# AlessioSam/LADiff

Hardware: AMD Instinct MI355X
Metric: motions/sec (196-frame, 50-step DDIM, bs128) (higher is better)
Workload: dtype f16x3+f32; 1 GPU; headline:ddim50_cfg7.5_b128_f196_c263_humanml3d; prompts_per_gpu=128, global_batch=128, frames=196, scheduler=ddim, denoising_steps=50, parallelism=dp1, loop=persistent pipeline kernel (16-row blocks x 86)

## Files before the change

ladiff_amd/build.py:

```python
import os
import subprocess
import sys
from concurrent.futures import ThreadPoolExecutor

HERE = os.path.dirname(os.path.abspath(__file__))
CSRC = os.path.join(HERE, "csrc")
OBJ = os.path.join(HERE, "csrc", "build")
LIB = os.path.join(HERE, "libladiff_hip.so")
SOURCES = ["gemm.hip", "gemm_big.hip", "gemm_kr.hip", "gemm_rowln.hip", "rowops.hip", "attention.hip", "qkv_attn.hip", "systolic.hip", "systolic_plan.hip", "linear_ca.hip", "dec_cross.hip", "dec_mlp.hip", "dec_qkv_attn.hip", "feats2joints.hip", "joint_metrics.hip", "vae_losses.hip", "denoiser.hip", "diffusion_stage.hip", "decoder.hip", "encoder.hip", "clip.hip", "evaluator.hip", "reverse.hip", "api.hip"]
FLAGS = ["--offload-arch=gfx950", "-O3", "-std=c++17", "-fPIC", "-fvisibility=hidden", "-Wall", "-Wno-unused-function"]


def _hipcc():
    for c in (os.environ.get("HIPCC"), "/opt/rocm/bin/hipcc", "hipcc"):
        if c and (os.path.isabs(c) and os.path.exists(c) or not os.path.isabs(c)):
            return c
    raise RuntimeError("hipcc not found")


def _stale(target, deps):
    if not os.path.exists(target):
        return True
    t = os.path.getmtime(target)
    return any(os.path.getmtime(d) > t for d in deps)


def stamps_lib(level=1):
    return LIB.replace(".so", "_stamps.so" if int(level) == 1 else f"_stamps{int(level)}.so")


def diag_lib():
    return LIB.replace(".so", "_diag.so")


def build(force=False, verbose=False, stamps=False, tag=None, defines=(), only=None):
    obj, lib, flags = OBJ, LIB, list(FLAGS)
    if tag:
        obj, lib = OBJ + "_" + tag, LIB.replace(".so", f"_{tag}.so")
        flags += ["-D" + d for d in defines]
    if stamps:
        lvl = os.environ.get("LADIFF_STAMPS_LEVEL", "1")
        obj, lib = OBJ + "_stamps" + (lvl if lvl != "1" else ""), stamps_lib(lvl)
        flags.append("-DLADIFF_STAMPS=" + lvl)
    os.makedirs(obj, exist_ok=True)
    headers = [os.path.join(CSRC, f) for f in os.listdir(CSRC) if f.endswith(".h")]
    headers += [os.path.join(os.path.dirname(HERE), "include", h) for h in ("ladiff_hip.h", "ladiff_hip_debug.h")]
    hipcc = _hipcc()
    jobs = []
    objdir = {src: (obj if only is None or src in only else OBJ) for src in SOURCES}
    for src in SOURCES:
        s = os.path.join(CSRC, src)
        o = os.path.join(objdir[src], src.replace(".hip", ".o"))
        if objdir[src] == obj and (force or _stale(o, [s] + headers)):
            jobs.append([hipcc, *flags, "-c", s, "-o", o])

    def run(cmd):
        if verbose:
            print(" ".join(cmd), flush=True)
        r = subprocess.run(cmd, capture_output=True, text=True)
        if r.returncode != 0:
            raise RuntimeError(f"hipcc failed: {' '.join(cmd)}\n{r.stdout}\n{r.stderr}")
        return r.stderr

    with ThreadPoolExecutor(max_workers=4) as ex:
        for err in ex.map(run, jobs):
            if verbose and err.strip():
                print(err)
    objs = [os.path.join(objdir[s], s.replace(".hip", ".o")) for s in SOURCES]
    if force or jobs or _stale(lib, objs + [os.path.join(CSRC, "exports.map")]):
        run([hipcc, "--offload-arch=gfx950", "-shared", "-fPIC", "-fvisibility=hidden", "-Wl,--version-script=" + os.path.join(CSRC, "exports.map"),
             "-o", lib, *objs])
    return lib


def build_all(force=False, verbose=False):
    lib = build(force=force, verbose=verbose)
    build(force=force, verbose=verbose, tag="bf16", defines=["LADIFF_SPLIT_BF16"])
    build(force=force, verbose=verbose, tag="diag", defines=["LADIFF_TAG_BITS=4", "LADIFF_SELFCHECK"], only=("systolic.hip",))
    return lib


if __name__ == "__main__":
    _tag = next((a.split("=", 1)[1] for a in sys.argv if a.startswith("--tag=")), None)
    _defs = [a[2:] for a in sys.argv if a.startswith("-D")]
    if "--all" in sys.argv:
        print(build_all(force="--force" in sys.argv, verbose=True))
    else:
        print(build(force="--force" in sys.argv, verbose=True, stamps="--stamps" in sys.argv, tag=_tag, defines=_defs))
```

ladiff_amd/csrc/api.hip:

```cpp
#include <algorithm>
#include <cstdlib>
#include <cstring>
#include <vector>

#include "model.h"
#include "sampler.h"
#include "../../include/ladiff_hip_debug.h"

using namespace ladiff;

namespace {

inline hipStream_t S(ladiff_stream_t s) { return reinterpret_cast<hipStream_t>(s); }

bool all_set(const float* const* w, size_t n) {
    if (w == nullptr) return false;
    for (size_t i = 0; i < n; ++i)
        if (w[i] == nullptr) return false;
    return true;
}
template <class W>
bool load_weights(W& dst, const float* const* ptrs) {
    if (!all_set(ptrs, sizeof(W) / sizeof(const float*))) return false;
    std::memcpy(&dst, ptrs, sizeof(W));
    return true;
}
const char* name_at(const std::vector<std::string>& n, int i) { return (i >= 0 && i < (int)n.size()) ? n[i].c_str() : nullptr; }

}

#ifdef LADIFF_STAMPS
static unsigned long long* g_stamps = nullptr;
#endif

extern "C" {

int ladiff_version(void) { return LADIFF_ABI_VERSION; }
int ladiff_split_format(void) {
#ifndef LADIFF_SPLIT_BF16
    return 1;
#else
    return 0;
#endif
}

const char* ladiff_error_string(int code) {
    switch (code) {
        case LADIFF_OK: return "ok";
        case LADIFF_ERR_ARG: return "invalid argument (null pointer or negative size)";
        case LADIFF_ERR_SHAPE: return "shape not supported by the gfx950 kernels";
        case LADIFF_ERR_WORKSPACE: return "workspace too small";
        case LADIFF_ERR_UNSUPPORTED: return "configuration branch not built";
        default: return code > 0 ? hipGetErrorString((hipError_t)code) : "unknown ladiff error";
    }
}

int ladiff_denoiser_num_params(void) { return DEN_NPARAMS; }
const char* ladiff_denoiser_param_name(int i) { return name_at(denoiser_param_names(), i); }
int ladiff_decoder_num_params(void) { return DEC_NPARAMS; }
const char* ladiff_decoder_param_name(int i) { return name_at(decoder_param_names(), i); }

int ladiff_gemm(const float* A, int lda, const float* A2, int lda2, int K1, const float* W, int ldw, const float* bias,
                const float* res, int ldres, const float* ln_gamma, const float* ln_beta, float* Y, int ldy, int M,
                int N, int K, int act, ladiff_stream_t stream) {
    LADIFF_CHECK_ARG(A && W && Y && M >= 0 && N > 0 && K > 0);
    GemmArgs g;
    g.A = A; g.lda = lda; g.A2 = A2; g.lda2 = lda2; g.K1 = A2 ? K1 : K; g.W = W; g.ldw = ldw; g.bias = bias;
    g.res = res; g.ldres = ldres; g.ln_g = ln_gamma; g.ln_b = ln_beta; g.Y = Y; g.ldy = ldy; g.M = M; g.N = N; g.K = K;
    g.act = act;
    return launch_gemm(g, S(stream));
}

int ladiff_gemm_resident(const float* A, int lda, const float* A2, int lda2, int K1, const float* W, int ldw,
                         const float* bias, const float* res, int ldres, float* Y, int ldy, int M, int N, int K, int act,
                         int split, float* Ys, ladiff_stream_t stream) {
    LADIFF_CHECK_ARG(A && W && (Y || Ys) && M >= 0 && N > 0 && K > 0);
    if (M == 0) return 0;
    KrArgs g;
    g.A = A; g.lda = lda; g.A2 = A2; g.lda2 = lda2; g.K1 = A2 ? K1 : K; g.W = W; g.ldw = ldw; g.bias = bias;
    g.res = res; g.ldres = ldres; g.Y = Y; g.ldy = ldy; g.M = M; g.N = N; g.K = K; g.act = act;
    g.split = split; g.Ys = Ys;
#ifdef LADIFF_STAMPS
    g.stamps = g_stamps;
#endif
    return launch_gemm_kr(g, S(stream));
}

int ladiff_gemm_split(const float* A, int lda, const float* A2, int lda2, int K1, const float* W, int ldw, const float* bias,
                      const float* res, int ldres, float* Y, float* Ys, int ldy, int M, int N, int K, int act,
                      ladiff_stream_t stream) {
    LADIFF_CHECK_ARG(A && W && (Y || Ys) && M >= 0 && N > 0 && K > 0);
    if (M == 0) return 0;
    GemmArgs g;
    g.A = A; g.lda = lda; g.A2 = A2; g.lda2 = lda2; g.K1 = A2 ? K1 : K; g.W = W; g.ldw = ldw; g.bias = bias;
    g.res = res; g.ldres = ldres; g.Y = Y; g.Ys = Ys; g.ldy = ldy; g.M = M; g.N = N; g.K = K; g.act = act; g.split = 1;
    return launch_gemm(g, S(stream));
}

#ifdef LADIFF_STAMPS
void ladiff_debug_set_stamps(unsigned long long* p) { g_stamps = p; }
void ladiff_debug_set_sys_stamps(unsigned long long* p) { ladiff::g_sys_stamps = p; }
void ladiff_debug_set_probe(int v) { ladiff::g_sys_probe = v; }
#endif

int ladiff_combine_rows(const float* partials, int n_planes, int M, const float* bias, const float* res, int mode,
                        const float* ln_gamma, const float* ln_beta, const float* table, const int32_t* counts, int Bs,
                        int T, int pad_row, float* out, ladiff_stream_t stream) {
    LADIFF_CHECK_ARG(partials && out && n_planes > 0 && M >= 0 && Bs > 0 && T > 0);
    if (mode != RED_PLAIN && mode != RED_LN && mode != RED_LN_ADD && mode != RED_LN_MOD) return LADIFF_ERR_ARG;
    if (mode != RED_PLAIN && !(ln_gamma && ln_beta)) return LADIFF_ERR_ARG;
    if ((mode == RED_LN_ADD || mode == RED_LN_MOD) && !table) return LADIFF_ERR_ARG;
    if (M == 0) return 0;
    return launch_reduce_rows(partials, n_planes, M, bias, res, mode, ln_gamma, ln_beta, table, 0, nullptr, counts, Bs, T,
                              pad_row, 0, out, nullptr, S(stream));
}

int ladiff_layernorm(const float* x, const float* gamma, const float* beta, float* y, int M, ladiff_stream_t stream) {
    LADIFF_CHECK_ARG(x && gamma && beta && y && M >= 0);
    return launch_layernorm(x, gamma, beta, y, M, S(stream));
}

int ladiff_timestep_sinusoid(const int64_t* timesteps, int n, float* out, ladiff_stream_t stream) {
    LADIFF_CHECK_ARG(timesteps && out && n >= 0);
    if (n == 0) return 0;
    return launch_sinusoid(timesteps, n, out, S(stream));
}

int ladiff_decoder_self_attention(const float* qkv, const int32_t* lengths, const uint32_t* keybits, float* out, int B,
                                  int F, ladiff_stream_t stream) {
    LADIFF_CHECK_ARG(qkv && (lengths || keybits) && out && B >= 0);
    return launch_decoder_self_attention(qkv, lengths, keybits, out, B, F, 0, S(stream));
}

int ladiff_self_attention_split(const float* qkv, const int32_t* lengths, const uint32_t* keybits, float* out, int B, int F,
                                 int nheads, int causal, ladiff_stream_t stream) {
    LADIFF_CHECK_ARG(qkv && out && B >= 0);
    return launch_self_attention_split(qkv, lengths, keybits, out, B, F, nheads, causal, 0, S(stream));
}

int ladiff_decoder_cross_attention(const float* q, const float* kv, const int32_t* counts, float* out, int B, int F,
                                   int T, ladiff_stream_t stream) {
    LADIFF_CHECK_ARG(q && kv && out && B >= 0 && F >= 0);
    return launch_decoder_cross_attention(q, kv, counts, out, B, F, T, 0, S(stream));
}

size_t ladiff_denoiser_tables_floats(int n_steps) { return den_tables_floats(n_steps); }
size_t ladiff_denoiser_text_cache_floats(int B2, int n_steps, int n_text) { return den_text_cache_floats(B2, n_steps, n_text); }
size_t ladiff_denoiser_workspace_bytes(int B2, int T, int n_steps, int n_text) {
    return sizeof(float) * std::max({den_forward_ws_floats(B2, T), den_time_layout(nullptr, n_steps).total,
                                     den_text_ws_floats(B2, n_steps, n_text), den_text_ws_floats(B2, n_steps, 1)});
}

int ladiff_denoiser_time_tables(const float* const* w, const float* sinusoid, int n_steps, float* tables, void* ws,
                                size_t ws_bytes, ladiff_stream_t stream) {
    DenoiserW W;
    LADIFF_CHECK_ARG(load_weights(W, w) && sinusoid && tables && ws && n_steps > 0);
    if (ws_bytes < ladiff_denoiser_workspace_bytes(1, 1, n_steps, 1)) return LADIFF_ERR_WORKSPACE;
    return denoiser_time_tables(W, sinusoid, n_steps, tables, (float*)ws, ws_bytes / sizeof(float), S(stream));
}

int ladiff_denoiser_text_cache(const float* const* w, const float* text_emb, int B2, int n_text, const float* tables, int n_steps,
                               float* cache, void* ws, size_t ws_bytes, ladiff_stream_t stream) {
    DenoiserW W;
    LADIFF_CHECK_ARG(load_weights(W, w) && text_emb && tables && cache && ws && B2 > 0 && n_steps > 0 && n_text >= 1);
    if (ws_bytes < ladiff_denoiser_workspace_bytes(B2, 1, n_steps, n_text)) return LADIFF_ERR_WORKSPACE;
    return denoiser_text_cache(W, text_emb, B2, tables, n_steps, cache, (float*)ws, ws_bytes / sizeof(float), S(stream), n_text);
}

int ladiff_denoiser_forward(const float* const* w, const float* const* w_split, const float* tables, const int32_t* d_step,
                            const float* text_cache, int n_text, int n_steps, const float* sample, int Bs, int dup, int T,
                            const int32_t* counts, float* eps, void* ws, size_t ws_bytes, ladiff_stream_t stream) {
    DenoiserW W, WS;
    LADIFF_CHECK_ARG(load_weights(W, w) && tables && d_step && text_cache && sample && eps && ws && Bs > 0 && dup > 0 && n_steps > 0 &&
                     n_text >= 1);
    if (w_split != nullptr) LADIFF_CHECK_ARG(load_weights(WS, w_split));
    if (T < 1 || T > LADIFF_MAX_LATENTS) return LADIFF_ERR_SHAPE;
    if (ws_bytes < ladiff_denoiser_workspace_bytes(Bs * dup, T, n_steps, n_text)) return LADIFF_ERR_WORKSPACE;
    return denoiser_forward(W, w_split ? &WS : nullptr, tables, d_step, text_cache, n_steps, sample, Bs, dup, T, counts, eps, (float*)ws,
                            ws_bytes / sizeof(float), S(stream), 0, -1, 0, n_text);
}

size_t ladiff_linear_cross_attention_workspace_bytes(int B, int T, int n_text) {
    return linear_cross_attention_ws_floats(B, T, n_text) * sizeof(float);
}
int ladiff_linear_cross_attention(const float* const* w, int layer, const float* x, const float* xf, const float* emb,
                                  const int32_t* counts, int B, int T, int n_text, float* out, void* ws, size_t ws_bytes,
                                  ladiff_stream_t stream) {
    DenoiserW W;
    LADIFF_CHECK_ARG(load_weights(W, w) && x && xf && emb && out && ws && B > 0);
    return linear_cross_attention(W, layer, x, xf, emb, counts, B, T, n_text, out, (float*)ws, ws_bytes / sizeof(float), S(stream));
}

int ladiff_cfg_scheduler_step(const float* eps, float* latents, const float* coef, const int32_t* d_step,
                              const float* step_noise, float guidance_scale, int cfg, int B, int T,
                              ladiff_stream_t stream) {
    LADIFF_CHECK_ARG(eps && latents && coef && d_step && B > 0 && T > 0);
    return launch_cfg_step(eps, latents, coef, d_step, step_noise, guidance_scale, cfg, B, T, S(stream));
}
int ladiff_advance_step(int32_t* d_step, ladiff_stream_t stream) {
    LADIFF_CHECK_ARG(d_step);
    return launch_advance(d_step, S(stream));
}
int ladiff_init_latents(const float* noise, const int32_t* counts, float sigma, float* latents, int B, int T,
                        ladiff_stream_t stream) {
    LADIFF_CHECK_ARG(noise && latents && B > 0 && T > 0);
    return launch_init_latents(noise, counts, sigma, latents, B, T, S(stream));
}
int ladiff_finalize_latents(const float* latents, const int32_t* counts, float* z, int B, int T, ladiff_stream_t stream) {
    LADIFF_CHECK_ARG(latents && z && B > 0 && T > 0);
    return launch_finalize_latents(latents, counts, z, B, T, S(stream));
}

int ladiff_sampler_create(void** sampler) {
    LADIFF_CHECK_ARG(sampler);
    *sampler = new Sampler();
    return 0;
}
int ladiff_sampler_destroy(void* sampler) {
    Sampler* sp = reinterpret_cast<Sampler*>(sampler);
    if (sp == nullptr) return 0;
    (void)hipDeviceSynchronize();
    sp->drain_retired();
    if (sp->exec) (void)hipGraphExecDestroy(sp->exec);
    if (sp->setup) (void)hipGraphExecDestroy(sp->setup);
    if (sp->ev0) (void)hipEventDestroy(sp->ev0);
    if (sp->ev1) (void)hipEventDestroy(sp->ev1);
    for (hipEvent_t e : sp->wev) (void)hipEventDestroy(e);
    sp->cap.destroy();
    delete sp;
    return 0;
}

int ladiff_reverse_plan(int B, int T, const int32_t* h_counts, int masked, int loop_mode, int f16x3, int cfg, int* rows_per_block, int* n_blocks) {
    LADIFF_CHECK_ARG(B >= 1 && T >= 1 && T <= LADIFF_MAX_LATENTS && loop_mode >= 1 && loop_mode <= 3 && rows_per_block && n_blocks);
    if (!cfg && masked && h_counts == nullptr) return LADIFF_ERR_UNSUPPORTED;
    std::vector<unsigned char> plan;
    int mr = 2, nb = 0;
    choose_plan(B, T, h_counts, masked != 0, loop_mode, f16x3 != 0, plan, &mr, &nb, cfg != 0);
    *rows_per_block = 16 * mr; *n_blocks = nb;
    return 0;
}

int ladiff_debug_set_stage_waves(int waves_per_simd) {
    LADIFF_CHECK_ARG(waves_per_simd == 1 || waves_per_simd == 2);
    g_waves16 = waves_per_simd;
    return 0;
}

int ladiff_debug_set_handoff(int tagged) {
    LADIFF_CHECK_ARG(tagged == 0 || tagged == 1);
    g_handoff = tagged;
    return 0;
}

int ladiff_debug_set_mlp_variant(int v) {
#ifdef LADIFF_STAMPS
    LADIFF_CHECK_ARG((v >= 0 && v <= 3) || (v >= 11 && v <= 17) || (v >= 21 && v <= 26));
#else
    LADIFF_CHECK_ARG(v >= 0 && v <= 3);
#endif
    g_mlp_variant = v;
    return 0;
}

int ladiff_debug_set_decoder_fusion(int on) {
    LADIFF_CHECK_ARG(on >= 0 && on <= 126 && (on & 3) != 3 && (on & 48) != 48);
    g_dec_out_cross = (on & 64) ? 0 : 1;
    g_dec_fused_mlp = on & 3;
    g_dec_small_rows_path = (on & 4) ? 0 : 1;
    g_dec_final_split = (on & 8) ? 0 : 1;
    g_dec_fused_attn = (on & 16) ? 0 : (on & 32) ? 2 : 1;
    return 0;
}

int ladiff_debug_set_stage_plan(int v) {
    LADIFF_CHECK_ARG(v >= 0 && v <= 1);
    g_stage_plan = v;
    return 0;
}

int ladiff_debug_set_poll_pause(int mask, int len) {
    LADIFF_CHECK_ARG(mask >= 0 && mask <= 255 && len >= 0 && len <= 64);
    g_poll_pause = mask | (len << 8);
    return 0;
}

int ladiff_debug_set_pacing(int eighths, int mask) {
    if (eighths == -1) { g_pace = -1; return 0; }
    LADIFF_CHECK_ARG(eighths >= 0 && eighths <= 8 && mask >= 0 && mask <= 255);
    g_pace = eighths | (mask << 8);
    return 0;
}

int ladiff_debug_set_stage_delay(int mask, int len) {
    LADIFF_CHECK_ARG(mask >= -1 && mask <= 255 && len >= 0 && len <= 64);
    g_stage_delay = mask < 0 ? -1 : (mask | (len << 8));
    return 0;
}

int ladiff_debug_set_loop_thresholds(int look_ahead_from, int small_upto) {
    LADIFF_CHECK_ARG(look_ahead_from >= -1 && small_upto >= -1);
    g_look_ahead_from = look_ahead_from;
    g_small_upto = small_upto;
    return 0;
}

int ladiff_debug_set_graph_epoch_rule(int on) {
    LADIFF_CHECK_ARG(on == 0 || on == 1);
    g_graph_epoch_rule = on;
    return 0;
}

int ladiff_debug_graph_instantiations(void) { return g_graph_instantiations.load(); }

int ladiff_debug_set_xcd_local(int on) {
    LADIFF_CHECK_ARG(on >= 0 && on <= 2);
    g_xcd_local = on;
    return 0;
}

int ladiff_sampler_set_loop(void* sampler, int mode) {
    Sampler* sp = reinterpret_cast<Sampler*>(sampler);
    LADIFF_CHECK_ARG(sp != nullptr && mode >= 0 && mode <= 3);
    sp->loop = mode != 0;
    sp->loop_mode = mode;
    return 0;
}

int ladiff_sampler_loop_ms(void* sampler, float* ms) {
    Sampler* sp = reinterpret_cast<Sampler*>(sampler);
    LADIFF_CHECK_ARG(sp != nullptr && ms != nullptr && sp->ev1 != nullptr);
    LADIFF_HIP(hipEventSynchronize(sp->ev1));
    LADIFF_HIP(hipEventElapsedTime(ms, sp->ev0, sp->ev1));
    return 0;
}

int ladiff_sampler_set_window_timing(void* sampler, int on) {
    Sampler* sp = reinterpret_cast<Sampler*>(sampler);
    LADIFF_CHECK_ARG(sp != nullptr);
    sp->time_windows = on != 0;
    return 0;
}

int ladiff_sampler_window_ms(void* sampler, float* loop_ms_sum, int* n_windows) {
    Sampler* sp = reinterpret_cast<Sampler*>(sampler);
    LADIFF_CHECK_ARG(sp != nullptr && loop_ms_sum != nullptr && n_windows != nullptr);
    float sum = 0.f;
    for (int i = 0; i < sp->n_windows; ++i) {
        float ms = 0.f;
        LADIFF_HIP(hipEventSynchronize(sp->wev[2 * i + 1]));
        LADIFF_HIP(hipEventElapsedTime(&ms, sp->wev[2 * i], sp->wev[2 * i + 1]));
        sum += ms;
    }
    *loop_ms_sum = sum; *n_windows = sp->n_windows;
    return 0;
}

int ladiff_sampler_last_loop(void* sampler, int* pipeline, int* rows_per_block, int* n_blocks) {
    Sampler* sp = reinterpret_cast<Sampler*>(sampler);
    LADIFF_CHECK_ARG(sp != nullptr && pipeline != nullptr);
    *pipeline = sp->last_pipeline;
    if (rows_per_block) *rows_per_block = sp->last_pipeline ? 16 * sp->plan_mr : 0;
    if (n_blocks) *n_blocks = sp->last_pipeline ? sp->plan_nb : 0;
    return 0;
}

int ladiff_sampler_set_noise_generator(void* sampler, uint64_t seed, uint32_t first_prompt, int enable) {
    Sampler* sp = reinterpret_cast<Sampler*>(sampler);
    LADIFF_CHECK_ARG(sp != nullptr);
    sp->gen = NoiseGen{(unsigned)(seed & 0xffffffffull), (unsigned)(seed >> 32), first_prompt, enable ? 1 : 0};
    return 0;
}

int ladiff_noise_fill(uint64_t seed, uint32_t first_prompt, int first_step, int n_steps, int B, int T, float* out, ladiff_stream_t stream) {
    LADIFF_CHECK_ARG(out != nullptr && first_step >= 0 && n_steps >= 0 && B >= 0);
    if (T < 1 || T > LADIFF_MAX_LATENTS) return LADIFF_ERR_SHAPE;
    return launch_noise_fill(NoiseGen{(unsigned)(seed & 0xffffffffull), (unsigned)(seed >> 32), first_prompt, 1}, first_step, n_steps, B, T, out,
                             S(stream));
}

int ladiff_sampler_set_fault(void* sampler, int workgroup, int timeout_ms) {
    Sampler* sp = reinterpret_cast<Sampler*>(sampler);
    LADIFF_CHECK_ARG(sp != nullptr && workgroup >= -1 && workgroup < 256 && timeout_ms >= 0);
    sp->fault_wg = workgroup;
    sp->timeout_ticks = (unsigned long long)timeout_ms * 100000ull;
    return 0;
}

size_t ladiff_reverse_status_offset_bytes(int B, int T, int n_steps, int n_text) {
    if (B < 1 || T < 1 || T > LADIFF_MAX_LATENTS || n_steps < 1 || n_text < 1) return 0;
    const ReverseWs r = carve_reverse(nullptr, B, T, n_steps, n_text);
    return (r.sys_off + sys_status_offset_floats(B, T)) * sizeof(float);
}

int ladiff_reverse_status(void* ws, int B, int T, int n_steps, int n_text, int* code, int* info) {
    LADIFF_CHECK_ARG(ws && code && B > 0 && n_steps > 0);
    if (T < 1 || T > LADIFF_MAX_LATENTS) return LADIFF_ERR_SHAPE;
    const ReverseWs r = carve_reverse(ws, B, T, n_steps, n_text);
    unsigned st[2] = {0u, 0u};
    LADIFF_HIP(hipMemcpy(st, r.sys + sys_status_offset_floats(B, T), sizeof(st), hipMemcpyDeviceToHost));
    *code = (int)st[0];
    if (info) *info = (int)st[1];
    return 0;
}

size_t ladiff_reverse_workspace_bytes(int B, int T, int n_steps, int n_text) { return carve_reverse(nullptr, B, T, n_steps, n_text).total_bytes; }

int ladiff_mlp_ln_fused(const float* xs, const float* x, const float* w1s, const float* b1, const float* w2s, const float* b2,
                        const float* ln_gamma, const float* ln_beta, const float* ln2_gamma, const float* ln2_beta, float* y, float* ys,
                        int M, ladiff_stream_t stream) {
    LADIFF_CHECK_ARG(xs && x && w1s && b1 && w2s && b2 && ln_gamma && ln_beta && (y || ys) && M >= 0);
    if ((ln2_gamma == nullptr) != (ln2_beta == nullptr)) return LADIFF_ERR_ARG;
    return launch_dec_mlp(xs, x, w1s, b1, w2s, b2, ln_gamma, ln_beta, ln2_gamma, ln2_beta, y, ys, M, S(stream));
}

int ladiff_split_rows(const float* x, float* y, int R, int K, ladiff_stream_t stream) {
    LADIFF_CHECK_ARG(x && y && R >= 0 && K > 0);
    if (K % 64) return LADIFF_ERR_SHAPE;
    if (R == 0) return 0;
    return launch_split_rows(x, y, R, K, S(stream));
}

int ladiff_gather_rows(const float* src, const int32_t* index, int n_rows, int row_floats, float* dst, ladiff_stream_t stream) {
    LADIFF_CHECK_ARG(n_rows >= 0 && row_floats > 0);
    if (n_rows == 0) return 0;
    LADIFF_CHECK_ARG(src && index && dst);
    if (row_floats % 4 || (reinterpret_cast<uintptr_t>(src) & 15) || (reinterpret_cast<uintptr_t>(dst) & 15)) return LADIFF_ERR_SHAPE;
    if ((reinterpret_cast<uintptr_t>(index) & 3) || n_rows > (1 << 30)) return LADIFF_ERR_SHAPE;
    return launch_gather_rows(src, index, n_rows, row_floats, dst, S(stream));
}

int ladiff_split_range_stats(const float* const* tensors, const int64_t* counts, int n, int64_t max_count, uint64_t* stats,
                             ladiff_stream_t stream) {
    LADIFF_CHECK_ARG(n >= 0 && max_count >= 0);
    if (n == 0) return 0;
    LADIFF_CHECK_ARG(tensors && counts && stats);
    if (n > 65535 || max_count >= (int64_t(1) << 32)) return LADIFF_ERR_SHAPE;
    return launch_split_range_stats(tensors, counts, n, max_count, reinterpret_cast<unsigned long long*>(stats), S(stream));
}

int ladiff_diffusion_reverse(void* sampler, const float* const* w, const float* const* w_split, uint64_t weights_generation,
                             const float* text_emb, const float* init_noise, const int32_t* counts, const int32_t* final_counts,
                             const int32_t* h_counts, const float* sinusoid, const float* coef, const float* step_noise, float guidance_scale,
                             float init_noise_sigma, int cfg, int B, int T, int n_text, int n_steps, float* z, void* ws, size_t ws_bytes,
                             int reuse_time_tables, ladiff_stream_t stream) {
    DenoiserW W, WS;
    LADIFF_CHECK_ARG(load_weights(W, w) && text_emb && init_noise && sinusoid && coef && z && ws && B > 0 && n_steps > 0);
    if (w_split != nullptr) LADIFF_CHECK_ARG(load_weights(WS, w_split));
    if (T < 1 || T > LADIFF_MAX_LATENTS || n_text < 1) return LADIFF_ERR_SHAPE;
    return diffusion_reverse(reinterpret_cast<Sampler*>(sampler), W, w_split ? &WS : nullptr,
                             ReverseArgs{w, w_split, weights_generation, text_emb, init_noise, counts, final_counts, h_counts, sinusoid, coef,
                                         step_noise, guidance_scale, init_noise_sigma, cfg, B, T, n_text, n_steps, z, ws, ws_bytes,
                                         reuse_time_tables, stream});
}

int ladiff_encoder_num_params(void) { return ENC_NPARAMS; }
const char* ladiff_encoder_param_name(int i) { return name_at(encoder_param_names(), i); }
size_t ladiff_encoder_workspace_bytes(int B, int F, int T, int C) { return enc_ws_floats(B, F, T, C) * sizeof(float); }

int ladiff_vae_encode(const float* const* w, const float* const* w_split, const float* features, const int32_t* lengths,
                      const int32_t* counts, const float* eps, int B, int F, int T, int C, float* mu, float* std,
                      float* latent, void* ws, size_t ws_bytes, ladiff_stream_t stream) {
    EncoderW W, WS;
    LADIFF_CHECK_ARG(load_weights(W, w) && features && lengths && counts && eps && mu && std && latent && ws && B >= 0);
    if (w_split != nullptr) LADIFF_CHECK_ARG(load_weights(WS, w_split));
    return vae_encode(W, w_split ? &WS : nullptr, features, lengths, counts, eps, B, F, T, C, mu, std, latent, (float*)ws,
                      ws_bytes / sizeof(float), S(stream));
}

int ladiff_vae_encode_dvae(const float* const* w, const float* const* w_split, const float* features, const int32_t* lengths,
                           const int32_t* counts, const float* eps, int B, int F, int T, int C, float* mu, float* std, float* latent,
                           void* ws, size_t ws_bytes, const int32_t* slot, const float* values, int n, ladiff_stream_t stream) {
    EncoderW W, WS;
    LADIFF_CHECK_ARG(load_weights(W, w) && features && lengths && counts && eps && mu && std && latent && ws && B >= 0);
    LADIFF_CHECK_ARG(slot && n >= 0 && (values || n == 0));
    if (w_split != nullptr) LADIFF_CHECK_ARG(load_weights(WS, w_split));
    if ((reinterpret_cast<uintptr_t>(slot) & 3) || (reinterpret_cast<uintptr_t>(values) & 3)) return LADIFF_ERR_SHAPE;
    return vae_encode(W, w_split ? &WS : nullptr, features, lengths, counts, eps, B, F, T, C, mu, std, latent, (float*)ws,
                      ws_bytes / sizeof(float), S(stream), slot, values, n);
}

size_t ladiff_vae_losses_workspace_bytes(int B, int F, int C, int J, int T) { return vae_losses_ws_floats(B, F, C, J, T) * sizeof(float); }

int ladiff_vae_losses(const float* m_rst, const float* m_ref, const float* joints_rst, const float* joints_ref, const float* mu,
                      const float* std, int B, int F, int C, int J, int T, double lambda_rec, double lambda_joint, double lambda_kl,
                      double* batch, double* acc, void* ws, size_t ws_bytes, ladiff_stream_t stream) {
    LADIFF_CHECK_ARG(m_rst && m_ref && joints_rst && joints_ref && mu && std && batch && acc && ws);
    if (B < 1 || F < 1 || C < 1 || J < 1 || T < 1) return LADIFF_ERR_SHAPE;
    for (const void* p : {(const void*)m_rst, (const void*)m_ref, (const void*)joints_rst, (const void*)joints_ref, (const void*)mu,
                          (const void*)std})
        if (reinterpret_cast<uintptr_t>(p) & 3) return LADIFF_ERR_SHAPE;
    for (const void* p : {(const void*)batch, (const void*)acc, (const void*)ws})
        if (reinterpret_cast<uintptr_t>(p) & 7) return LADIFF_ERR_SHAPE;
    const VaeLossWs a = vae_losses_layout((float*)ws, B, F, C, J, T);
    if (ws_bytes / sizeof(float) < a.total) return LADIFF_ERR_WORKSPACE;
    return launch_vae_losses(m_rst, m_ref, (size_t)B * F * C, joints_rst, joints_ref, (size_t)B * F * J * 3, mu, std, (size_t)T * B * D,
                             lambda_rec, lambda_joint, lambda_kl, a.part, a.blocks, batch, acc, S(stream));
}

size_t ladiff_denoiser_forward_timesteps_workspace_bytes(int B2, int T) { return den_per_sample_ws_floats(B2, T) * sizeof(float); }

int ladiff_denoiser_forward_timesteps(const float* const* w, const float* const* w_split, const float* text_emb, int n_text,
                                      const int64_t* timesteps, const float* sample, int B2, int T, const int32_t* counts, float* eps,
                                      void* ws, size_t ws_bytes, ladiff_stream_t stream) {
    DenoiserW W, WS;
    LADIFF_CHECK_ARG(load_weights(W, w) && text_emb && timesteps && sample && eps && ws);
    if (w_split != nullptr) LADIFF_CHECK_ARG(load_weights(WS, w_split));
    if (n_text != 1) return LADIFF_ERR_UNSUPPORTED;
    if (B2 < 1 || T < 1 || T > LADIFF_MAX_LATENTS) return LADIFF_ERR_SHAPE;
    for (const void* p : {(const void*)text_emb, (const void*)sample, (const void*)eps, (const void*)ws})
        if (reinterpret_cast<uintptr_t>(p) & 15) return LADIFF_ERR_SHAPE;
    if ((reinterpret_cast<uintptr_t>(timesteps) & 7) || (reinterpret_cast<uintptr_t>(counts) & 3)) return LADIFF_ERR_SHAPE;
    if (ws_bytes < ladiff_denoiser_forward_timesteps_workspace_bytes(B2, T)) return LADIFF_ERR_WORKSPACE;
    return denoiser_forward_timesteps(W, w_split ? &WS : nullptr, text_emb, timesteps, sample, B2, T, counts, eps, (float*)ws,
                                      ws_bytes / sizeof(float), S(stream));
}

int ladiff_q_sample(const float* z, const int64_t* timesteps, const float* alphas_cumprod, int n_train, const int32_t* counts, int draw,
                    uint64_t seed, uint32_t first_prompt, float* noise, float* noisy, int B, int T, ladiff_stream_t stream) {
    LADIFF_CHECK_ARG(z && timesteps && alphas_cumprod && noise && noisy && n_train > 0);
    if (B < 1 || T < 1 || T > LADIFF_MAX_LATENTS) return LADIFF_ERR_SHAPE;
    for (const void* p : {(const void*)z, (const void*)noise, (const void*)noisy})
        if (reinterpret_cast<uintptr_t>(p) & 15) return LADIFF_ERR_SHAPE;
    if ((reinterpret_cast<uintptr_t>(timesteps) & 7) || (reinterpret_cast<uintptr_t>(alphas_cumprod) & 3) ||
        (reinterpret_cast<uintptr_t>(counts) & 3))
        return LADIFF_ERR_SHAPE;
    return launch_q_sample(z, timesteps, alphas_cumprod, n_train, counts,
                           NoiseGen{(unsigned)(seed & 0xffffffffull), (unsigned)(seed >> 32), first_prompt, draw ? 1 : 0}, noise, noisy, B, T,
                           S(stream));
}

size_t ladiff_diffusion_losses_workspace_bytes(int64_t n) { return n < 1 ? 0 : diffusion_losses_layout(nullptr, (size_t)n).total * sizeof(float); }

int ladiff_diffusion_losses(const float* noise_pred, const float* noise, int64_t n, double lambda_inst, double* batch, double* acc, void* ws,
                            size_t ws_bytes, ladiff_stream_t stream) {
    LADIFF_CHECK_ARG(noise_pred && noise && batch && acc && ws);
    if (n < 1) return LADIFF_ERR_SHAPE;
    if ((reinterpret_cast<uintptr_t>(noise_pred) & 3) || (reinterpret_cast<uintptr_t>(noise) & 3)) return LADIFF_ERR_SHAPE;
    for (const void* p : {(const void*)batch, (const void*)acc, (const void*)ws})
        if (reinterpret_cast<uintptr_t>(p) & 7) return LADIFF_ERR_SHAPE;
    const DiffLossWs a = diffusion_losses_layout((float*)ws, (size_t)n);
    if (ws_bytes / sizeof(float) < a.total) return LADIFF_ERR_WORKSPACE;
    return launch_diffusion_losses(noise_pred, noise, (size_t)n, lambda_inst, a.part, a.blocks, batch, acc, S(stream));
}

int ladiff_clip_num_params(void) { return CLIP_NPARAMS; }
const char* ladiff_clip_param_name(int i) { return name_at(clip_param_names(), i); }
size_t ladiff_clip_workspace_bytes(int B, int L) { return clip_ws_floats(B, L) * sizeof(float); }

static bool load_clip(ClipW& dst, const float* const* ptrs, int n_layers) {
    if (ptrs == nullptr || n_layers < 1 || n_layers > CLIP_MAX_LAYERS) return false;
    const int n = CLIP_HEAD_NPARAMS + CLIP_LAYER_NPARAMS * n_layers;
    for (int i = 0; i < n; ++i)
        if (ptrs[i] == nullptr) return false;
    std::memset(&dst, 0, sizeof(dst));
    std::memcpy(&dst, ptrs, n * sizeof(const float*));
    return true;
}

int ladiff_clip_text_encode(const float* const* w, const float* const* w_split, int n_layers, int vocab, const int64_t* ids,
                            int B, int seq, int L, float* out, void* ws, size_t ws_bytes, ladiff_stream_t stream) {
    ClipW W, WS;
    LADIFF_CHECK_ARG(load_clip(W, w, n_layers) && ids && out && ws && B >= 0);
    if (w_split != nullptr) LADIFF_CHECK_ARG(load_clip(WS, w_split, n_layers));
    return clip_text_encode(W, w_split ? &WS : nullptr, n_layers, vocab, ids, B, seq, L, out, (float*)ws,
                            ws_bytes / sizeof(float), S(stream));
}

size_t ladiff_clip_workspace_bytes_ragged(int B, int total_rows) { return clip_ws_floats_rows(B, total_rows) * sizeof(float); }

int ladiff_clip_text_encode_ragged(const float* const* w, const float* const* w_split, int n_layers, int vocab, const int64_t* ids,
                                   int B, int seq, int L, const int32_t* seq_len, const int32_t* row_off, const int32_t* row_seq,
                                   int total_rows, float* out, void* ws, size_t ws_bytes, ladiff_stream_t stream) {
    ClipW W, WS;
    LADIFF_CHECK_ARG(load_clip(W, w, n_layers) && ids && out && ws && B >= 0 && seq_len && row_off && row_seq && total_rows >= 0);
    if (w_split != nullptr) LADIFF_CHECK_ARG(load_clip(WS, w_split, n_layers));
    return clip_text_encode(W, w_split ? &WS : nullptr, n_layers, vocab, ids, B, seq, L, out, (float*)ws,
                            ws_bytes / sizeof(float), S(stream), seq_len, row_off, row_seq, total_rows);
}

int ladiff_t2m_movement_num_params(void) { return (int)t2m_move_param_names().size(); }
const char* ladiff_t2m_movement_param_name(int i) { return name_at(t2m_move_param_names(), i); }
int ladiff_t2m_motion_num_params(void) { return (int)t2m_motion_param_names().size(); }
const char* ladiff_t2m_motion_param_name(int i) { return name_at(t2m_motion_param_names(), i); }
int ladiff_t2m_text_num_params(void) { return (int)t2m_text_param_names().size(); }
const char* ladiff_t2m_text_param_name(int i) { return name_at(t2m_text_param_names(), i); }
size_t ladiff_t2m_movement_workspace_bytes(int B, int F, int Cin) { return t2m_move_ws_floats(B, F, Cin) * sizeof(float); }
size_t ladiff_t2m_motion_workspace_bytes(int B, int T) { return t2m_motion_ws_floats(B, T) * sizeof(float); }
size_t ladiff_t2m_text_workspace_bytes(int B, int L) { return t2m_text_ws_floats(B, L) * sizeof(float); }

int ladiff_t2m_movement_encode(const float* const* w, const float* feats, int ld, int B, int F, int Cin, float* out, void* ws,
                               size_t ws_bytes, ladiff_stream_t stream) {
    LADIFF_CHECK_ARG(all_set(w, t2m_move_param_names().size()) && feats && out && ws && B >= 0);
    return t2m_movement_encode(w, feats, ld, B, F, Cin, out, (float*)ws, ws_bytes / sizeof(float), S(stream));
}
int ladiff_t2m_motion_encode(const float* const* w, const float* movements, const int32_t* m_lens, int B, int T, float* out,
                             void* ws, size_t ws_bytes, ladiff_stream_t stream) {
    LADIFF_CHECK_ARG(all_set(w, t2m_motion_param_names().size()) && movements && m_lens && out && ws && B >= 0);
    return t2m_motion_encode(w, movements, m_lens, B, T, out, (float*)ws, ws_bytes / sizeof(float), S(stream));
}
int ladiff_t2m_text_encode(const float* const* w, const float* word_embs, const float* pos_onehot, const int32_t* cap_lens,
                           int B, int L, float* out, void* ws, size_t ws_bytes, ladiff_stream_t stream) {
    LADIFF_CHECK_ARG(all_set(w, t2m_text_param_names().size()) && word_embs && pos_onehot && cap_lens && out && ws && B >= 0);
    return t2m_text_encode(w, word_embs, pos_onehot, cap_lens, B, L, out, (float*)ws, ws_bytes / sizeof(float), S(stream));
}

int ladiff_feats2joints(const float* feats, const float* mean, const float* std, int B, int F, int C, int njoints,
                        float* joints, ladiff_stream_t stream) {
    LADIFF_CHECK_ARG(feats && mean && std && joints && B >= 0);
    return launch_feats2joints(feats, mean, std, B, F, C, njoints, joints, S(stream));
}

namespace {
int joint_metrics_check(const void* rst, const void* ref, const int32_t* h_lengths, int B, int F, int J, const void* seq_rows, const void* acc) {
    if (J != 21 && J != 22) return LADIFF_ERR_SHAPE;
    if (F < 1 || F > LADIFF_MAX_FRAMES) return LADIFF_ERR_SHAPE;
    for (int b = 0; b < B; ++b)
        if (h_lengths[b] < 1 || h_lengths[b] > F) return LADIFF_ERR_SHAPE;
    if ((reinterpret_cast<uintptr_t>(rst) & 3) || (reinterpret_cast<uintptr_t>(ref) & 3) || (reinterpret_cast<uintptr_t>(seq_rows) & 3) ||
        (reinterpret_cast<uintptr_t>(acc) & 7))
        return LADIFF_ERR_SHAPE;
    return 0;
}
}

int ladiff_joint_ape_ave(const float* joints_rst, const float* joints_ref, const int32_t* lengths, const int32_t* h_lengths, int B, int F,
                         int J, const int32_t* h_part_idx, float factor, float* seq_rows, double* acc, ladiff_stream_t stream) {
    LADIFF_CHECK_ARG(B >= 0);
    if (B == 0) return 0;
    LADIFF_CHECK_ARG(joints_rst && joints_ref && lengths && h_lengths && h_part_idx && seq_rows && acc && factor > 0.f);
    LADIFF_TRY(joint_metrics_check(joints_rst, joints_ref, h_lengths, B, F, J, seq_rows, acc));
    if (reinterpret_cast<uintptr_t>(lengths) & 3) return LADIFF_ERR_SHAPE;
    for (int i = 0; i < 8; ++i)
        if (h_part_idx[i] < 0 || h_part_idx[i] >= (i < 4 ? J - 1 : J)) return LADIFF_ERR_SHAPE;
    return launch_joint_ape_ave(joints_rst, joints_ref, lengths, B, F, J, h_part_idx, factor, seq_rows, acc, S(stream));
}

int ladiff_joint_mr(const float* joints_rst, const float* joints_ref, const int32_t* h_lengths, int B, int F, int J, float* seq_rows,
                    double* acc, ladiff_stream_t stream) {
    LADIFF_CHECK_ARG(B >= 0);
    if (B == 0) return 0;
    LADIFF_CHECK_ARG(joints_rst && joints_ref && h_lengths && seq_rows && acc);
    LADIFF_TRY(joint_metrics_check(joints_rst, joints_ref, h_lengths, B, F, J, seq_rows, acc));
    return launch_joint_mr(joints_rst, joints_ref, B, F, J, seq_rows, acc, S(stream));
}

size_t ladiff_decoder_workspace_bytes(int B, int F, int T, int C) {
    (void)C;
    return dec_ws_floats(B, (size_t)B * F, T) * sizeof(float);
}

int ladiff_vae_decode(const float* const* w, const float* const* w_split, const float* z, const int32_t* lengths,
                      const int32_t* counts, int B, int F, int T, int C, float* feats, void* ws, size_t ws_bytes,
                      ladiff_stream_t stream) {
    DecoderW W, WS;
    LADIFF_CHECK_ARG(load_weights(W, w) && z && lengths && feats && ws && B >= 0);
    if (w_split != nullptr) LADIFF_CHECK_ARG(load_weights(WS, w_split));
    return vae_decode(W, w_split ? &WS : nullptr, z, lengths, counts, nullptr, 0, B, F, T, C, feats, (float*)ws, ws_bytes / sizeof(float),
                      S(stream));
}

namespace {
struct DecodeGraph {
    hipGraphExec_t exec = nullptr;
    GraphSlot slot;
    CaptureStream cap;
};
}

int ladiff_decoder_graph_create(void** graph) {
    LADIFF_CHECK_ARG(graph);
    *graph = new DecodeGraph();
    return 0;
}
int ladiff_decoder_graph_destroy(void* graph) {
    DecodeGraph* g = reinterpret_cast<DecodeGraph*>(graph);
    if (g == nullptr) return 0;
    (void)hipDeviceSynchronize();
    if (g->exec) (void)hipGraphExecDestroy(g->exec);
    g->cap.destroy();
    delete g;
    return 0;
}

int ladiff_vae_decode_graphed(void* graph, const float* const* w, const float* const* w_split, uint64_t weights_generation, const float* z,
                              const int32_t* lengths, const int32_t* counts, const int32_t* row_off, int total_rows, int B, int F, int T,
                              int C, float* feats, void* ws, size_t ws_bytes, ladiff_stream_t stream) {
    DecodeGraph* dg = reinterpret_cast<DecodeGraph*>(graph);
    DecoderW W, WS;
    LADIFF_CHECK_ARG(dg && load_weights(W, w) && z && lengths && feats && ws && B >= 0 && stream != nullptr);
    if (w_split != nullptr) LADIFF_CHECK_ARG(load_weights(WS, w_split));
    if (F < 1 || F > LADIFF_MAX_FRAMES || T < 1 || T > LADIFF_MAX_LATENTS || C < 1) return LADIFF_ERR_SHAPE;
    if (ws_bytes < ladiff_decoder_workspace_bytes(B, F, T, C)) return LADIFF_ERR_WORKSPACE;
    hipStream_t s = S(stream);
    const GraphKey key = decode_key(w, w_split, DEC_NPARAMS, weights_generation, z, lengths, counts, row_off, total_rows, B, F, T, C, feats, ws,
                                    stream, g_dec_fused_mlp, g_dec_small_rows_path, g_dec_final_split, g_mlp_variant, g_dec_fused_attn);
    if (!(dg->exec && dg->slot.key == key && dg->slot.newest())) {
        if (dg->exec) { LADIFF_HIP(hipStreamSynchronize(s)); (void)hipGraphExecDestroy(dg->exec); dg->exec = nullptr; }
        LADIFF_TRY(dec_mlp_prepare());
        LADIFF_TRY(dec_qkv_attn_prepare());
        LADIFF_TRY(dec_cross_prepare());
        LADIFF_TRY(dg->cap.ensure());
        LADIFF_TRY(capture_graph(dg->cap.s, [&](hipStream_t cs) {
            if (row_off != nullptr) LADIFF_TRY(launch_zero_fill(feats, (size_t)B * F * C, cs));
            return vae_decode(W, w_split ? &WS : nullptr, z, lengths, counts, row_off, total_rows, B, F, T, C, feats, (float*)ws,
                              ws_bytes / sizeof(float), cs);
        }, &dg->exec));
        dg->slot.stamp(key);
    }
    LADIFF_HIP(hipGraphLaunch(dg->exec, s));
    return 0;
}

int ladiff_vae_decode_ragged(const float* const* w, const float* const* w_split, const float* z, const int32_t* lengths,
                             const int32_t* counts, const int32_t* row_off, int total_rows, int B, int F, int T, int C, float* feats,
                             void* ws, size_t ws_bytes, ladiff_stream_t stream) {
    DecoderW W, WS;
    LADIFF_CHECK_ARG(load_weights(W, w) && z && lengths && row_off && feats && ws && B >= 0 && total_rows >= 0);
    if (w_split != nullptr) LADIFF_CHECK_ARG(load_weights(WS, w_split));
    if (F < 1 || F > LADIFF_MAX_FRAMES || T < 1 || T > LADIFF_MAX_LATENTS || C < 1) return LADIFF_ERR_SHAPE;
    if (ws_bytes < ladiff_decoder_workspace_bytes(B, F, T, C)) return LADIFF_ERR_WORKSPACE;
    LADIFF_HIP(hipMemsetAsync(feats, 0, (size_t)B * F * C * sizeof(float), S(stream)));
    return vae_decode(W, w_split ? &WS : nullptr, z, lengths, counts, row_off, total_rows, B, F, T, C, feats, (float*)ws,
                      ws_bytes / sizeof(float), S(stream));
}

}
```

ladiff_amd/csrc/dec_cross.hip:

```cpp
#include <mutex>
#include "kernels.h"
#include "tile_mma.h"

namespace ladiff { extern unsigned long long* g_sys_stamps; }

namespace ladiff {

namespace {
constexpr int TM = LADIFF_MAX_LATENTS;
}

__global__ __launch_bounds__(256) void dec_cross_prep_kernel(const DecCrossPrepBatch pb, int B, int T, int tiles_per_wg) {
    const int h = blockIdx.y, layer = blockIdx.z, tid = threadIdx.x, lane = tid & 63, c16 = lane & 15, kq = lane >> 4;
    const int wave = __builtin_amdgcn_readfirstlane(tid >> 6);
    const float* __restrict__ kv = pb.kv[layer]; const float* __restrict__ wq = pb.wq[layer]; const float* __restrict__ bq = pb.bq[layer];
    const float* __restrict__ wo = pb.wo[layer]; float* __restrict__ gu = pb.gu[layer];
    float* __restrict__ cc = gu + (size_t)B * H * T * 2 * D;
    const int M = T * B, ntiles = (M + 15) / 16;
    float gq[4][16], uo[4][16], bqv[16];
#pragma unroll
    for (int t = 0; t < 4; ++t) {
        const int n = 64 * wave + 16 * t + c16;
#pragma unroll
        for (int s = 0; s < 16; ++s) gq[t][s] = wq[(size_t)(h * DH + 16 * kq + s) * D + n];
#pragma unroll
        for (int s4 = 0; s4 < 16; s4 += 4) {
            const f32x4 w4 = ld4(wo + (size_t)n * D + h * DH + 16 * kq + s4);
#pragma unroll
            for (int e = 0; e < 4; ++e) uo[t][s4 + e] = w4[e];
        }
    }
#pragma unroll
    for (int s4 = 0; s4 < 16; s4 += 4) {
        const f32x4 b4 = ld4(bq + h * DH + 16 * kq + s4);
#pragma unroll
        for (int e = 0; e < 4; ++e) bqv[s4 + e] = b4[e];
    }
    const int tile1 = (blockIdx.x + 1) * tiles_per_wg < ntiles ? (blockIdx.x + 1) * tiles_per_wg : ntiles;
    for (int tile = blockIdx.x * tiles_per_wg; tile < tile1; ++tile) {
        const int arow = 16 * tile + c16 < M ? 16 * tile + c16 : M - 1;
        const float* kr = kv + (size_t)arow * 2 * D + h * DH + 16 * kq;
        float ak[16], av[16];
#pragma unroll
        for (int s4 = 0; s4 < 16; s4 += 4) {
            const f32x4 k4 = ld4(kr + s4), v4 = ld4(kr + D + s4);
#pragma unroll
            for (int e = 0; e < 4; ++e) { ak[s4 + e] = k4[e]; av[s4 + e] = v4[e]; }
        }
        f32x4 ag[4], au[4];
#pragma unroll
        for (int t = 0; t < 4; ++t) { ag[t] = f32x4{0.f, 0.f, 0.f, 0.f}; au[t] = ag[t]; }
#pragma unroll
        for (int s = 0; s < 16; ++s)
#pragma unroll
            for (int t = 0; t < 4; ++t) {
                ag[t] = __builtin_amdgcn_mfma_f32_16x16x4f32(ak[s], gq[t][s], ag[t], 0, 0, 0);
                au[t] = __builtin_amdgcn_mfma_f32_16x16x4f32(av[s], uo[t][s], au[t], 0, 0, 0);
            }
#pragma unroll
        for (int i = 0; i < 4; ++i) {
            const int bt = 16 * tile + 4 * kq + i;
            if (bt < M) {
                const int j = bt / B, b = bt - j * B;
                float* o = gu + ((((size_t)b * H + h) * T + j) * 2) * D + 64 * wave + c16;
#pragma unroll
                for (int t = 0; t < 4; ++t) { o[16 * t] = ag[t][i] * 0.125f; o[D + 16 * t] = au[t][i]; }
            }
        }
        if (wave == 0) {
            float c = 0.f;
#pragma unroll
            for (int s = 0; s < 16; ++s) c = fmaf(bqv[s], ak[s], c);
            c += __shfl_xor(c, 16, 64); c += __shfl_xor(c, 32, 64);
            const int bt = 16 * tile + c16;
            if (kq == 0 && bt < M) { const int j = bt / B, b = bt - j * B; cc[((size_t)b * H + h) * T + j] = c * 0.125f; }
        }
    }
}

template <int T>
__device__ __forceinline__ void cross_row(const f32x4 (&xv)[4], f32x4 (&acc)[4], const float* sm, const float* cs, int nv, int c0) {
#pragma unroll 1
    for (int h = 0; h < H; ++h) {
        float sc[T];
#pragma unroll
        for (int j = 0; j < T; ++j) {
            const float* gp = sm + ((size_t)(h * T + j) * 2) * D + c0;
            float d = 0.f;
#pragma unroll
            for (int k = 0; k < 4; ++k) {
                const f32x4 g4 = ld4(gp + 64 * k);
                d = fmaf(xv[k][0], g4[0], fmaf(xv[k][1], g4[1], fmaf(xv[k][2], g4[2], fmaf(xv[k][3], g4[3], d))));
            }
            sc[j] = d;
        }
#pragma unroll
        for (int j = 0; j < T; ++j) sc[j] = row16_sum(sc[j]) + cs[h * T + j];
        float m = -INFINITY;
#pragma unroll
        for (int j = 0; j < T; ++j) { sc[j] = j < nv ? sc[j] : -INFINITY; m = fmaxf(m, sc[j]); }
        float l = 0.f;
#pragma unroll
        for (int j = 0; j < T; ++j) { sc[j] = __builtin_amdgcn_exp2f((sc[j] - m) * 1.4426950408889634f); l += sc[j]; }
        const float inv = 1.f / l;
#pragma unroll
        for (int j = 0; j < T; ++j) {
            const float pj = sc[j] * inv;
            const float* up = sm + ((size_t)(h * T + j) * 2 + 1) * D + c0;
#pragma unroll
            for (int k = 0; k < 4; ++k) {
                const f32x4 u4 = ld4(up + 64 * k);
                acc[k][0] = fmaf(pj, u4[0], acc[k][0]); acc[k][1] = fmaf(pj, u4[1], acc[k][1]);
                acc[k][2] = fmaf(pj, u4[2], acc[k][2]); acc[k][3] = fmaf(pj, u4[3], acc[k][3]);
            }
        }
    }
}

template <int TT>
__global__ __launch_bounds__(256) void dec_cross_apply_kernel(const float* __restrict__ x, const float* __restrict__ gu,
                                                              const float* __restrict__ cc, const int32_t* __restrict__ counts,
                                                              const float* __restrict__ bo, const float* __restrict__ g2,
                                                              const float* __restrict__ b2, int F, int rows_per_wg,
                                                              float* __restrict__ y, float* __restrict__ ys,
                                                              const int32_t* __restrict__ row_off, const float* __restrict__ g1,
                                                              const float* __restrict__ b1) {
    extern __shared__ __attribute__((aligned(16))) float sm[];
    constexpr int T = TT, HT = H * TT;
    const int b = blockIdx.x, tid = threadIdx.x, lane = tid & 63, wave = tid >> 6;
    const float* src = gu + (size_t)b * HT * 2 * D;
    for (int u = tid; u < HT * 2 * D / 4; u += 256) st4(sm + 4 * u, ld4(src + 4 * u));
    float* cs = sm + (size_t)HT * 2 * D;
    if (tid < HT) cs[tid] = cc[(size_t)b * HT + tid];
    int nv = counts != nullptr ? counts[b] : T;
    nv = nv > T ? T : nv;
    __syncthreads();
    const int l16 = lane & 15, grp = lane >> 4, c0 = 4 * l16;
    f32x4 bo4[4], gg[4], bb[4];
#pragma unroll
    for (int k = 0; k < 4; ++k) { bo4[k] = ld4(bo + c0 + 64 * k); gg[k] = ld4(g2 + c0 + 64 * k); bb[k] = ld4(b2 + c0 + 64 * k); }
    size_t row0 = (size_t)b * F;
    if (row_off != nullptr) { row0 = row_off[b]; F = row_off[b + 1] - row_off[b]; }
    const int f0 = blockIdx.y * rows_per_wg;
    const int f1 = f0 + rows_per_wg < F ? f0 + rows_per_wg : F;
    for (int fb = f0; fb < f1; fb += 16) {
        const int f = fb + 4 * wave + grp;
        const bool live = f < f1;
        const size_t row = row0 + (live ? f : f1 - 1);
        f32x4 xv[4], acc[4];
#pragma unroll
        for (int k = 0; k < 4; ++k) xv[k] = ld4(x + row * D + c0 + 64 * k);
        if (g1 != nullptr) {
            float s1 = 0.f;
#pragma unroll
            for (int k = 0; k < 4; ++k) s1 += (xv[k][0] + xv[k][1]) + (xv[k][2] + xv[k][3]);
            const float mean1 = row16_sum(s1) * (1.f / 256.f);
            float q1 = 0.f;
#pragma unroll
            for (int k = 0; k < 4; ++k)
#pragma unroll
                for (int i = 0; i < 4; ++i) { const float dlt = xv[k][i] - mean1; q1 += dlt * dlt; }
            const float rstd1 = rsqrtf(row16_sum(q1) * (1.f / 256.f) + LN_EPS);
#pragma unroll
            for (int k = 0; k < 4; ++k) {
                const f32x4 ga = ld4(g1 + c0 + 64 * k), be = ld4(b1 + c0 + 64 * k);
#pragma unroll
                for (int i = 0; i < 4; ++i) xv[k][i] = (xv[k][i] - mean1) * rstd1 * ga[i] + be[i];
            }
        }
#pragma unroll
        for (int k = 0; k < 4; ++k)
#pragma unroll
            for (int i = 0; i < 4; ++i) acc[k][i] = bo4[k][i] + xv[k][i];
        cross_row<T>(xv, acc, sm, cs, nv, c0);
        float sum = 0.f;
#pragma unroll
        for (int k = 0; k < 4; ++k) sum += (acc[k][0] + acc[k][1]) + (acc[k][2] + acc[k][3]);
        const float mean = row16_sum(sum) * (1.f / 256.f);
        float q = 0.f;
#pragma unroll
        for (int k = 0; k < 4; ++k)
#pragma unroll
            for (int i = 0; i < 4; ++i) { const float dlt = acc[k][i] - mean; q += dlt * dlt; }
        const float rstd = rsqrtf(row16_sum(q) * (1.f / 256.f) + LN_EPS);
        if (live) {
#pragma unroll
            for (int k = 0; k < 4; ++k) {
                f32x4 o;
#pragma unroll
                for (int i = 0; i < 4; ++i) o[i] = (acc[k][i] - mean) * rstd * gg[k][i] + bb[k][i];
                st4(y + row * D + c0 + 64 * k, o);
                if (ys != nullptr) store_split4(ys + row * D, c0 + 64 * k, o);
            }
        }
    }
}


constexpr int OC_ROWS = 32;
constexpr int OC_TILE = OC_ROWS * 1024;
constexpr int OC_CT = OC_ROWS * CLD * 4;
constexpr int OC_XN = OC_ROWS * CLD * 4;
constexpr int OC_SLD = 36;
constexpr int OC_PS = 8 * OC_ROWS * OC_SLD * 4;
constexpr int OC_PT = OC_ROWS * 256;

struct OutCrossArgs {
    const float* att;
    const float* x0;
    const float* wo;
    const float* bo; const float* g1; const float* b1;
    const float* gu; const float* cc;
    const float* bo_c; const float* g2; const float* b2;
    const int32_t* counts; const int32_t* row_off;
    float* y; float* ys;
    int F, rows_per_wg;
    unsigned long long* stamps;
};

#ifdef LADIFF_STAMPS
#define OC_STAMP(i) do { if (p.stamps != nullptr && blockIdx.x == 3 && blockIdx.y == 0 && threadIdx.x == 0 && npass < 6) p.stamps[npass * 16 + (i)] = __builtin_amdgcn_s_memrealtime(); } while (0)
#else
#define OC_STAMP(i) do { } while (0)
#endif

__device__ __forceinline__ void oc_barrier() { asm volatile("s_waitcnt lgkmcnt(0)\n\ts_barrier" ::: "memory"); }

template <int TT>
__global__ __launch_bounds__(512, 1) void dec_out_cross_kernel(const OutCrossArgs p) {
    __shared__ __attribute__((aligned(1024))) char tile[OC_TILE];
    __shared__ __attribute__((aligned(1024))) char ps_b[OC_PS];
    __shared__ __attribute__((aligned(1024))) char ct_b[OC_CT];
    __shared__ __attribute__((aligned(1024))) char xn_b[OC_XN];
    __shared__ __attribute__((aligned(16))) float sc[OC_ROWS * OC_SLD];
    __shared__ __attribute__((aligned(256))) char ptile[OC_PT];
    __shared__ __attribute__((aligned(16))) float vec[6 * D];
    __shared__ float cs[32];
    constexpr int T = TT, HT = H * TT;
    static_assert(HT <= 32, "the (head, token) columns fit one k-step");
    float* ct = reinterpret_cast<float*>(ct_b);
    float* xn = reinterpret_cast<float*>(xn_b);
    float* ps = reinterpret_cast<float*>(ps_b);
    const int b = blockIdx.x, tid = threadIdx.x, lane = tid & 63, frow = lane & 15, fk = lane >> 4;
    const int wave = __builtin_amdgcn_readfirstlane(tid >> 6);
    int npass = 0;
    OC_STAMP(15);
    WFrag<0, 2, 1> gf, uf;
    {
        const float* gub = p.gu + (size_t)b * HT * 2 * D;
#pragma unroll
        for (int j = 0; j < 2; ++j) {
            const int hj = 16 * j + frow;
            f32x4 a = {0.f, 0.f, 0.f, 0.f}, c = a;
            if (hj < HT) { const float* g = gub + (size_t)hj * 2 * D + 32 * wave + 8 * fk; a = ld4(g); c = ld4(g + 4); }
            split8(a, c, gf.hi[j][0], gf.lo[j][0]);
            const int col = 32 * wave + 16 * j + frow;
            f32x4 u0 = {0.f, 0.f, 0.f, 0.f}, u1 = u0;
#pragma unroll
            for (int e = 0; e < 4; ++e) {
                if (8 * fk + e < HT) u0[e] = gub[((size_t)(8 * fk + e) * 2 + 1) * D + col];
                if (8 * fk + 4 + e < HT) u1[e] = gub[((size_t)(8 * fk + 4 + e) * 2 + 1) * D + col];
            }
            split8(u0, u1, uf.hi[j][0], uf.lo[j][0]);
        }
        if (tid < 32) cs[tid] = tid < HT ? p.cc[(size_t)b * HT + tid] : 0.f;
        const float* vs[6] = {p.bo, p.g1, p.b1, p.bo_c, p.g2, p.b2};
        if (tid < 6 * (D / 4)) st4(vec + 4 * tid, ld4(vs[tid / (D / 4)] + 4 * (tid % (D / 4))));
    }
    WFrag<0, 2, 8> wf;
    {
#pragma unroll 1
        for (int half = 0; half < 2; ++half) {
            if (half == 1) __syncthreads();
#pragma unroll
            for (int qq = 0; qq < 4; ++qq) {
                const int q = (qq + b) & 3;
                char* dst = q == 0 ? tile : q == 1 ? ps_b : q == 2 ? ct_b : xn_b;
#pragma unroll
                for (int kk = 0; kk < 4; ++kk) {
                    const int lr32 = wave + 8 * kk, r = 32 * q + lr32;
                    const char* src = reinterpret_cast<const char*>(p.wo) + ((size_t)(128 * half + r) << 10) + ((lane & 48) << 4) + ((((lane & 15) ^ r) & 15) << 4);
                    __builtin_amdgcn_global_load_lds(reinterpret_cast<const float*>(src), (__attribute__((address_space(3))) void*)(dst + lr32 * 1024), 16, 0, 0);
                }
            }
            __builtin_amdgcn_s_waitcnt(0xF70);
            __syncthreads();
            if ((wave >> 2) == half) {
                const int q = wave & 3;
                const char* srcb = q == 0 ? tile : q == 1 ? ps_b : q == 2 ? ct_b : xn_b;
#pragma unroll
                for (int j = 0; j < 2; ++j)
#pragma unroll
                    for (int st = 0; st < 8; ++st) {
                        const int r = 16 * j + frow;
                        wf.hi[j][st] = *reinterpret_cast<const s16x8*>(a_slot<4>(const_cast<char*>(srcb), r, st >> 1, 4 * (st & 1) + fk));
                        wf.lo[j][st] = *reinterpret_cast<const s16x8*>(a_slot<4>(const_cast<char*>(srcb), r, st >> 1, 8 + 4 * (st & 1) + fk));
                    }
            }
        }
        __syncthreads();
    }
    int nv = p.counts != nullptr ? p.counts[b] : T;
    nv = nv > T ? T : nv;
    int F = p.F;
    size_t row0 = (size_t)b * F;
    if (p.row_off != nullptr) { row0 = p.row_off[b]; F = p.row_off[b + 1] - p.row_off[b]; }
    const int f0 = blockIdx.y * p.rows_per_wg;
    const int f1 = f0 + p.rows_per_wg < F ? f0 + p.rows_per_wg : F;
    if (f0 >= f1) return;
    const int l16 = lane & 15, grp = lane >> 4, c0 = 4 * l16, lr = 4 * wave + grp;
    typedef unsigned u32x4_o __attribute__((ext_vector_type(4)));
    const float* x0s = ps;
    auto dma_att = [&](int fb) {
#pragma unroll
        for (int i = 0; i < 4; ++i) {
            const int r = wave + 8 * i, f = fb + r < f1 ? fb + r : f1 - 1;
            unsigned vo = ((lane & 48) << 4) + ((((lane & 15) ^ r) & 15) << 4);
            asm volatile("" : "+v"(vo));
            const char* src = reinterpret_cast<const char*>(p.att) + ((row0 + f) << 10) + vo;
            __builtin_amdgcn_global_load_lds(reinterpret_cast<const float*>(src), (__attribute__((address_space(3))) void*)(tile + r * 1024), 16, 0, 0);
        }
    };
    auto dma_x0 = [&](int fb) {
#pragma unroll
        for (int i = 0; i < 4; ++i) {
            const int r = wave + 8 * i, f = fb + r < f1 ? fb + r : f1 - 1;
            unsigned vo = lane << 4;
            asm volatile("" : "+v"(vo));
            const char* src = reinterpret_cast<const char*>(p.x0) + ((row0 + f) << 10) + vo;
            __builtin_amdgcn_global_load_lds(reinterpret_cast<const float*>(src), (__attribute__((address_space(3))) void*)(ps_b + r * 1024), 16, 0, 0);
        }
    };
    dma_att(f0);
    dma_x0(f0);
    __builtin_amdgcn_s_waitcnt(0xF70);
    __syncthreads();
    for (int fb = f0; fb < f1; fb += OC_ROWS, ++npass) {
        OC_STAMP(0);
        OC_STAMP(1);
        f32x4 acc2[2][2];
        zero_acc(acc2);
        mma<0, 4, 2, 8, 2>(tile, wf, acc2);
        OC_STAMP(2);
        const int f = fb + lr;
        const bool live = f < f1;
        const size_t row = row0 + (live ? f : f1 - 1);
        f32x4 xv[4];
        stage_c(ct, acc2, [&](int j) { return 32 * wave + 16 * j; });
        __builtin_amdgcn_s_waitcnt(0xF70);
        __syncthreads();
        OC_STAMP(3);
        {
            const float* cr = ct + lr * CLD + c0;
#pragma unroll
            for (int k = 0; k < 4; ++k) {
                const f32x4 o = ld4(cr + 64 * k), bo = ld4(vec + c0 + 64 * k), r0 = ld4(x0s + lr * D + c0 + 64 * k);
#pragma unroll
                for (int i = 0; i < 4; ++i) xv[k][i] = (o[i] + bo[i]) + r0[i];
            }
            float s1 = 0.f;
#pragma unroll
            for (int k = 0; k < 4; ++k) s1 += (xv[k][0] + xv[k][1]) + (xv[k][2] + xv[k][3]);
            const float mean1 = row16_sum(s1) * (1.f / 256.f);
            float q1 = 0.f;
#pragma unroll
            for (int k = 0; k < 4; ++k)
#pragma unroll
                for (int i = 0; i < 4; ++i) { const float dlt = xv[k][i] - mean1; q1 += dlt * dlt; }
            const float rstd1 = rsqrtf(row16_sum(q1) * (1.f / 256.f) + LN_EPS);
#pragma unroll
            for (int k = 0; k < 4; ++k) {
                const f32x4 ga = ld4(vec + D + c0 + 64 * k), be = ld4(vec + 2 * D + c0 + 64 * k);
#pragma unroll
                for (int i = 0; i < 4; ++i) xv[k][i] = (xv[k][i] - mean1) * rstd1 * ga[i] + be[i];
                st4(xn + lr * CLD + c0 + 64 * k, xv[k]);
                tile_put4<0, 4>(tile, lr, c0 + 64 * k, xv[k]);
            }
        }
        OC_STAMP(4);
        __syncthreads();
        OC_STAMP(5);
        {
            u32x4_o ah[2], al[2];
#pragma unroll
            for (int i = 0; i < 2; ++i) {
                ah[i] = *reinterpret_cast<const u32x4_o*>(a_slot<4>(tile, 16 * i + frow, wave >> 1, 4 * (wave & 1) + fk));
                al[i] = *reinterpret_cast<const u32x4_o*>(a_slot<4>(tile, 16 * i + frow, wave >> 1, 8 + 4 * (wave & 1) + fk));
            }
            f32x4 as[2][2];
            zero_acc(as);
#pragma unroll
            for (int i = 0; i < 2; ++i)
#pragma unroll
                for (int j = 0; j < 2; ++j) as[i][j] = MFMA16_S16(__builtin_bit_cast(s16x8, al[i]), gf.hi[j][0], as[i][j], 0, 0, 0);
#pragma unroll
            for (int i = 0; i < 2; ++i)
#pragma unroll
                for (int j = 0; j < 2; ++j) as[i][j] = MFMA16_S16(__builtin_bit_cast(s16x8, ah[i]), gf.lo[j][0], as[i][j], 0, 0, 0);
#pragma unroll
            for (int i = 0; i < 2; ++i)
#pragma unroll
                for (int j = 0; j < 2; ++j) as[i][j] = MFMA16_S16(__builtin_bit_cast(s16x8, ah[i]), gf.hi[j][0], as[i][j], 0, 0, 0);
            float* pw = ps + wave * (OC_ROWS * OC_SLD);
#pragma unroll
            for (int i = 0; i < 2; ++i)
#pragma unroll
                for (int j = 0; j < 2; ++j)
#pragma unroll
                    for (int r = 0; r < 4; ++r) pw[(16 * i + 4 * fk + r) * OC_SLD + 16 * j + frow] = as[i][j][r];
        }
        __syncthreads();
        OC_STAMP(6);
        if (fb + OC_ROWS < f1) dma_att(fb + OC_ROWS);
        {
            float tot[2];
#pragma unroll
            for (int u = 0; u < 2; ++u) {
                const int hj = 16 * u + l16;
                float a = 0.f;
#pragma unroll
                for (int w = 0; w < 8; ++w) a += ps[w * (OC_ROWS * OC_SLD) + lr * OC_SLD + hj];
                tot[u] = a + cs[hj];
                sc[lr * OC_SLD + hj] = tot[u];
            }
            asm volatile("s_waitcnt lgkmcnt(0)" ::: "memory");
            __builtin_amdgcn_wave_barrier();
            float hs[2][T];
            int hh[2], jj[2];
#pragma unroll
            for (int u = 0; u < 2; ++u) {
                const int hj = 16 * u + l16;
                hh[u] = hj < HT ? hj / T : 0; jj[u] = hj - hh[u] * T;
#pragma unroll
                for (int t = 0; t < T; ++t) hs[u][t] = sc[lr * OC_SLD + hh[u] * T + t];
            }
#pragma unroll
            for (int u = 0; u < 2; ++u) {
                const int hj = 16 * u + l16;
                float m = -INFINITY, l = 0.f;
#pragma unroll
                for (int t = 0; t < T; ++t) m = t < nv ? fmaxf(m, hs[u][t]) : m;
#pragma unroll
                for (int t = 0; t < T; ++t) l += t < nv ? __builtin_amdgcn_exp2f((hs[u][t] - m) * 1.4426950408889634f) : 0.f;
                float pr = __builtin_amdgcn_exp2f((tot[u] - m) * 1.4426950408889634f) / l;
                if (!(hj < HT && jj[u] < nv)) pr = 0.f;
                tile_put1<0, 1>(ptile, lr, hj, pr);
            }
        }
        oc_barrier();
        OC_STAMP(7);
        f32x4 ao[2][2];
        zero_acc(ao);
        mma<0, 1, 2, 1, 2>(ptile, uf, ao);
        stage_c(ct, ao, [&](int j) { return 32 * wave + 16 * j; });
        __builtin_amdgcn_s_waitcnt(0xF70);
        oc_barrier();
        OC_STAMP(8);
        {
            const float* cr = ct + lr * CLD + c0;
            f32x4 acc[4];
#pragma unroll
            for (int k = 0; k < 4; ++k) {
                const f32x4 o = ld4(cr + 64 * k), bc = ld4(vec + 3 * D + c0 + 64 * k), x1 = ld4(xn + lr * CLD + c0 + 64 * k);
#pragma unroll
                for (int i = 0; i < 4; ++i) acc[k][i] = (bc[i] + x1[i]) + o[i];
            }
            if (fb + OC_ROWS < f1) dma_x0(fb + OC_ROWS);
            float sum = 0.f;
#pragma unroll
            for (int k = 0; k < 4; ++k) sum += (acc[k][0] + acc[k][1]) + (acc[k][2] + acc[k][3]);
            const float mean = row16_sum(sum) * (1.f / 256.f);
            float q = 0.f;
#pragma unroll
            for (int k = 0; k < 4; ++k)
#pragma unroll
                for (int i = 0; i < 4; ++i) { const float dlt = acc[k][i] - mean; q += dlt * dlt; }
            const float rstd = rsqrtf(row16_sum(q) * (1.f / 256.f) + LN_EPS);
            if (live) {
#pragma unroll
                for (int k = 0; k < 4; ++k) {
                    const f32x4 ga = ld4(vec + 4 * D + c0 + 64 * k), be = ld4(vec + 5 * D + c0 + 64 * k);
                    f32x4 o;
#pragma unroll
                    for (int i = 0; i < 4; ++i) o[i] = (acc[k][i] - mean) * rstd * ga[i] + be[i];
                    st4(p.y + row * D + c0 + 64 * k, o);
                    if (p.ys != nullptr) store_split4(p.ys + row * D, c0 + 64 * k, o);
                }
            }
        }
        OC_STAMP(9);
    }
}

int dec_cross_prepare() {
    static std::mutex mu;
    static bool attr_set[64] = {};
    int dev = 0;
    LADIFF_HIP(hipGetDevice(&dev));
    if (dev < 0 || dev >= 64) return LADIFF_ERR_ARG;
    std::lock_guard<std::mutex> lock(mu);
    if (!attr_set[dev]) {
        LADIFF_HIP(hipFuncSetAttribute(reinterpret_cast<const void*>(dec_cross_apply_kernel<8>), hipFuncAttributeMaxDynamicSharedMemorySize,
                                       (int)(((size_t)H * TM * 2 * D + H * TM) * sizeof(float))));
        const void* oc[8] = {reinterpret_cast<const void*>(dec_out_cross_kernel<1>), reinterpret_cast<const void*>(dec_out_cross_kernel<2>),
                             reinterpret_cast<const void*>(dec_out_cross_kernel<3>), reinterpret_cast<const void*>(dec_out_cross_kernel<4>),
                             reinterpret_cast<const void*>(dec_out_cross_kernel<5>), reinterpret_cast<const void*>(dec_out_cross_kernel<6>),
                             reinterpret_cast<const void*>(dec_out_cross_kernel<7>), reinterpret_cast<const void*>(dec_out_cross_kernel<8>)};
        for (int t = 1; t <= 8; ++t)
            (void)oc[t - 1];
        attr_set[dev] = true;
    }
    return 0;
}

int launch_decoder_cross_prep(const DecCrossPrepBatch& pb, int n, int B, int T, hipStream_t s) {
    if (B == 0 || n == 0) return 0;
    if (T < 1 || T > TM || n > DEC_PREP_MAX) return LADIFF_ERR_SHAPE;
    const int ntiles = (T * B + 15) / 16;
    int tpw = 1;
    while (tpw < 8 && (ntiles + 2 * tpw - 1) / (2 * tpw) * H * n >= 160) tpw *= 2;
    hipLaunchKernelGGL(dec_cross_prep_kernel, dim3((ntiles + tpw - 1) / tpw, H, n), dim3(256), 0, s, pb, B, T, tpw);
    LADIFF_LAUNCH_CHECK();
    return 0;
}

int launch_decoder_cross_apply(const float* x, const float* bo, const float* g2, const float* b2, const int32_t* counts, int B, int F,
                               int T, const float* gu_ws, float* y, float* ys, hipStream_t s, const int32_t* row_off, const float* g1,
                               const float* b1) {
    if (B == 0 || F == 0) return 0;
    if (T < 1 || T > TM) return LADIFF_ERR_SHAPE;
    const float* gu = gu_ws;
    const float* cc = gu_ws + (size_t)B * H * T * 2 * D;
    int chunks = (512 + B - 1) / B;
    if (chunks < 1) chunks = 1;
    if (chunks > (F + 3) / 4) chunks = (F + 3) / 4;
    const int rows_per_wg = ((F + chunks - 1) / chunks + 15) / 16 * 16;
    chunks = (F + rows_per_wg - 1) / rows_per_wg;
    const size_t lds = ((size_t)H * T * 2 * D + H * T) * sizeof(float);
    LADIFF_TRY(dec_cross_prepare());
#define LADIFF_DC_CASE(TT)                                                                                                   \
    case TT:                                                                                                                 \
        hipLaunchKernelGGL(dec_cross_apply_kernel<TT>, dim3(B, chunks), dim3(256), lds, s, x, gu, cc, counts, bo, g2, b2, F, \
                           rows_per_wg, y, ys, row_off, g1, b1);                                                                              \
        break;
    switch (T) {
        LADIFF_DC_CASE(1) LADIFF_DC_CASE(2) LADIFF_DC_CASE(3) LADIFF_DC_CASE(4)
        LADIFF_DC_CASE(5) LADIFF_DC_CASE(6) LADIFF_DC_CASE(7) LADIFF_DC_CASE(8)
        default: return LADIFF_ERR_SHAPE;
    }
#undef LADIFF_DC_CASE
    LADIFF_LAUNCH_CHECK();
    return 0;
}

int launch_decoder_out_cross(const float* att_s, const float* x0, const float* wo_s, const float* bo, const float* g1, const float* b1,
                             const float* bo_c, const float* g2, const float* b2, const int32_t* counts, int B, int F, int T,
                             const float* gu_ws, float* y, float* ys, hipStream_t s, const int32_t* row_off) {
    if (B == 0 || F == 0) return 0;
    if (T < 1 || T > TM) return LADIFF_ERR_SHAPE;
    int chunks = (256 + B - 1) / B;
    if (chunks > (F + OC_ROWS - 1) / OC_ROWS) chunks = (F + OC_ROWS - 1) / OC_ROWS;
    if (chunks < 1) chunks = 1;
    const int rows_per_wg = ((F + chunks - 1) / chunks + OC_ROWS - 1) / OC_ROWS * OC_ROWS;
    chunks = (F + rows_per_wg - 1) / rows_per_wg;
    LADIFF_TRY(dec_cross_prepare());
    OutCrossArgs a{att_s, x0, wo_s, bo, g1, b1, gu_ws, gu_ws + (size_t)B * H * T * 2 * D, bo_c, g2, b2, counts, row_off, y, ys, F, rows_per_wg, nullptr};
#ifdef LADIFF_STAMPS
    a.stamps = g_sys_stamps;
#endif
#define LADIFF_OC_CASE(TT) \
    case TT: hipLaunchKernelGGL(dec_out_cross_kernel<TT>, dim3(B, chunks), dim3(512), 0, s, a); break;
    switch (T) {
        LADIFF_OC_CASE(1) LADIFF_OC_CASE(2) LADIFF_OC_CASE(3) LADIFF_OC_CASE(4)
        LADIFF_OC_CASE(5) LADIFF_OC_CASE(6) LADIFF_OC_CASE(7) LADIFF_OC_CASE(8)
        default: return LADIFF_ERR_SHAPE;
    }
#undef LADIFF_OC_CASE
    LADIFF_LAUNCH_CHECK();
    return 0;
}

}
```

ladiff_amd/csrc/dec_mlp.hip:

```cpp
#include <mutex>
#include "model.h"
#include "tile_mma.h"

namespace ladiff {

namespace {

constexpr int MLP_NS = 8;
constexpr int MLP_GRP = 4;
constexpr int MLP_STAGE = 16384;
constexpr int MLP_LDS = MLP_NS * MLP_STAGE + FF * 4 + 5 * D * 4;

typedef unsigned u32x4_m __attribute__((ext_vector_type(4)));

struct MlpArgs {
    const float* xs;
    const float* x;
    const float* w1;
    const float* b1;
    const float* w2;
    const float* b2;
    const float* g3; const float* be3;
    const float* g4; const float* be4;
    float* y; float* ys;
    int M;
};

__device__ __forceinline__ int pi_row(int p) { const int j = p >> 4, n = p & 15; return 32 * (j >> 1) + 8 * (n >> 2) + 4 * (j & 1) + (n & 3); }

template <int N> __device__ __forceinline__ void wait_vm() { asm volatile("s_waitcnt vmcnt(%0)" ::"n"(N) : "memory"); }
template <int OFF>
__device__ __forceinline__ void fetch16(u32x4_m& v, unsigned addr) {
    asm volatile("ds_read_b128 %0, %1 offset:%2" : "=v"(v) : "v"(addr), "n"(OFF) : "memory");
}
template <int OFF>
__device__ __forceinline__ void fetch16_keep(u32x4_m& v, unsigned addr) {
    asm volatile("ds_read_b128 %0, %1 offset:%2" : "+v"(v) : "v"(addr), "n"(OFF) : "memory");
}
template <int N>
__device__ __forceinline__ void wait_lgkm(u32x4_m& a, u32x4_m& b, u32x4_m& c, u32x4_m& d) {
    asm volatile("s_waitcnt lgkmcnt(%4)" : "+v"(a), "+v"(b), "+v"(c), "+v"(d) : "n"(N));
}
__device__ __forceinline__ s16x8 as_bf(const u32x4_m v) { return __builtin_bit_cast(s16x8, v); }

}

template <int NW, int RT, int DIAG = 0>
__global__ __launch_bounds__(64 * NW, NW / 4) void dec_mlp_kernel(const MlpArgs p) {
    constexpr int NT = 64 * NW, RW = 16 * RT, BM = RW * NW, PPW = 16 / NW;
    extern __shared__ __attribute__((aligned(1024))) char lds[];
    float* const b1s = reinterpret_cast<float*>(lds + MLP_NS * MLP_STAGE);
    const int tid = threadIdx.x, lane = tid & 63;
    const int wave = __builtin_amdgcn_readfirstlane(tid >> 6);
    const int frow = lane & 15, fk = lane >> 4;
    const int M = p.M;
    int myrow[RT]; bool live[RT];
#pragma unroll
    for (int rt = 0; rt < RT; ++rt) {
        myrow[rt] = blockIdx.x * BM + RW * wave + 16 * rt + frow;
        live[rt] = myrow[rt] < M;
        myrow[rt] = live[rt] ? myrow[rt] : M - 1;
    }

    s16x8 xh[RT][8], xl[RT][8];
#pragma unroll
    for (int rt = 0; rt < RT; ++rt) {
        const char* xr = reinterpret_cast<const char*>(p.xs) + (size_t)myrow[rt] * 1024 + fk * 16;
#pragma unroll
        for (int s = 0; s < 8; ++s) {
            xh[rt][s] = *reinterpret_cast<const s16x8*>(xr + (s >> 1) * 256 + (s & 1) * 64);
            xl[rt][s] = *reinterpret_cast<const s16x8*>(xr + (s >> 1) * 256 + (s & 1) * 64 + 128);
        }
    }
    for (int i = tid; i < FF / 4; i += NT) st4(b1s + 4 * i, ld4(p.b1 + 4 * i));
    float* const prm = b1s + FF;
    for (int i = tid; i < 5 * D / 4; i += NT) {
        const int which = i / (D / 4), c4 = i % (D / 4);
        const float* src = which == 0 ? p.b2 : which == 1 ? p.g3 : which == 2 ? p.be3 : which == 3 ? p.g4 : p.be4;
        if (src != nullptr) st4(prm + 4 * i, ld4(src + 4 * c4));
    }

    const int cs = (lane & 7) ^ ((lane >> 4) & 3) ^ (4 * (wave & 1));
    const int koff = (cs < 4 ? cs * 4 : 32 + (cs - 4) * 4);
    int src[PPW];
#pragma unroll
    for (int i = 0; i < PPW; ++i) src[i] = pi_row(8 * (wave + NW * i) + (lane >> 3));
    char* const dma_dst = lds + (8 * wave) * 128;
    auto issue = [&](int hs, auto uc, auto slotc, auto ic) __attribute__((always_inline)) {
        constexpr int u = decltype(uc)::value, slot = decltype(slotc)::value, i = decltype(ic)::value;
        const float* base; int ldw, n0, kb, half;
        const int hsv = hs < 0 ? 0 : hs;
        if constexpr (u < 8) { base = p.w1; ldw = D; n0 = 128 * hsv; kb = u >> 1; half = u & 1; }
        else { constexpr int v = u - 8, c = v >> 1; base = p.w2; ldw = FF; n0 = 128 * (v & 1); kb = 2 * hsv + (c >> 1); half = c & 1; }
        const float* s0 = base + (size_t)(n0 + src[i]) * ldw + kb * 64 + half * 16 + koff;
        if constexpr (DIAG == 1) { if (hs >= 0) return; }
        __builtin_amdgcn_global_load_lds(s0, (__attribute__((address_space(3))) void*)(dma_dst + slot * MLP_STAGE + 8 * NW * i * 128), 16, 0, 0);
    };

    const int sw = (frow >> 1) & 7;
    const unsigned rd_hi = lds_addr(lds) + frow * 128 + ((fk ^ sw) << 4);
    const unsigned rd_lo = lds_addr(lds) + frow * 128 + (((4 + fk) ^ sw) << 4);
    const unsigned rd_hi2 = rd_hi + 4 * MLP_STAGE, rd_lo2 = rd_lo + 4 * MLP_STAGE;

    f32x4 hacc[RT][8], oacc[RT][16];
    s16x8 hh[RT][4], hl[RT][4];
#pragma unroll
    for (int rt = 0; rt < RT; ++rt)
#pragma unroll
        for (int j = 0; j < 16; ++j) oacc[rt][j] = f32x4{0.f, 0.f, 0.f, 0.f};

    u32x4_m wt[4][2];
    u32x4_m dummy[4][2];
    if constexpr (DIAG == 3 || DIAG == 6 || DIAG == 7) {
#pragma unroll
        for (int i = 0; i < 4; ++i) { asm volatile("" : "=v"(wt[i][0])); asm volatile("" : "=v"(wt[i][1])); asm volatile("" : "=v"(dummy[i][0])); asm volatile("" : "=v"(dummy[i][1])); }
    }
    auto fetch_tile = [&](auto slotc, auto jc) __attribute__((always_inline)) {
        constexpr int slot = decltype(slotc)::value, j = decltype(jc)::value;
        if constexpr (DIAG == 3) return;
        const unsigned ah = slot < 4 ? rd_hi : rd_hi2, al = slot < 4 ? rd_lo : rd_lo2;
        constexpr int so = (slot & 3) * MLP_STAGE;
        if constexpr (DIAG == 6) { fetch16_keep<so + j * 2048>(dummy[j & 3][0], ah); fetch16_keep<so + j * 2048>(dummy[j & 3][1], al); return; }
        fetch16<so + j * 2048>(wt[j & 3][0], ah); fetch16<so + j * 2048>(wt[j & 3][1], al);
    };
    auto stage_mma = [&](auto slotc, auto& acc, auto j0c, const s16x8 (&bh)[RT], const s16x8 (&bl)[RT], auto&& between, auto&& next) __attribute__((always_inline)) {
        constexpr int slot = decltype(slotc)::value, J0 = decltype(j0c)::value;
        static_for<8>([&](auto jc) {
            constexpr int j = decltype(jc)::value, cur = j & 3;
            next(jc);
            if constexpr (DIAG != 3 && DIAG != 6) asm volatile("s_waitcnt lgkmcnt(4)" : "+v"(wt[cur][0]), "+v"(wt[cur][1]));
            __builtin_amdgcn_sched_barrier(0);
            static_for<3 * RT>([&](auto mc) {
                constexpr int m = decltype(mc)::value, prod = m / RT, rt = m % RT;
                if constexpr (DIAG == 7) {
                    acc[rt][J0 + j] = MFMA16_S16(as_bf(dummy[cur][prod == 1]), prod == 0 ? bl[rt] : bh[rt], acc[rt][J0 + j], 0, 0, 0);
                } else if constexpr (DIAG != 2) {
                    if constexpr (prod == 0) acc[rt][J0 + j] = MFMA16_S16(as_bf(wt[cur][0]), bl[rt], acc[rt][J0 + j], 0, 0, 0);
                    else if constexpr (prod == 1) acc[rt][J0 + j] = MFMA16_S16(as_bf(wt[cur][1]), bh[rt], acc[rt][J0 + j], 0, 0, 0);
                    else acc[rt][J0 + j] = MFMA16_S16(as_bf(wt[cur][0]), bh[rt], acc[rt][J0 + j], 0, 0, 0);
                }
                if constexpr (m == 0) {
                    __builtin_amdgcn_sched_barrier(0);
                    if constexpr (j + 3 < 8) fetch_tile(slotc, IntC<j + 3>{});
                    else fetch_tile(IntC<(slot + 1) % MLP_NS>{}, IntC<j + 3 - 8>{});
                    __builtin_amdgcn_sched_barrier(0);
                }
            });
            if constexpr (DIAG == 2) acc[0][J0 + j][0] += __builtin_bit_cast(float, wt[cur][0][0]) + __builtin_bit_cast(float, wt[cur][1][1]);
            __builtin_amdgcn_sched_barrier(0);
            if constexpr (j & 1) between(IntC<j / 2>{});
        });
    };

    static_for<MLP_GRP>([&](auto uc) {
        constexpr int u = decltype(uc)::value;
        static_for<PPW>([&](auto ic) { issue(DIAG == 1 ? -1 : 0, IntC<u>{}, IntC<u>{}, ic); });
    });
    __syncthreads();
    auto landed = [&]() __attribute__((always_inline)) {
        wait_vm<0>();
        __builtin_amdgcn_s_barrier();
    };
    landed();
    static_for<PPW>([&](auto ic) { issue(DIAG == 1 ? -1 : 0, IntC<MLP_GRP>{}, IntC<MLP_GRP>{}, ic); });
    static_for<3>([&](auto jc) { fetch_tile(IntC<0>{}, jc); });
    constexpr int H = PPW / 2;
#pragma unroll 1
    for (int hs = 0; hs < 8; ++hs) {
        static_for<16>([&](auto uc) {
            constexpr int u = decltype(uc)::value, slot = u % MLP_NS, r = u % MLP_GRP;
            auto batch_pieces = [&](auto aheadc, auto halfc) __attribute__((always_inline)) {
                constexpr int ahead = decltype(aheadc)::value, half = decltype(halfc)::value;
                constexpr int ut = (u + ahead) % 16, slot_t = (u + ahead) % MLP_NS;
                const int hs_t = (hs + (u + ahead >= 16 ? 1 : 0)) & 7;
                static_for<H>([&](auto ic) { issue(hs_t, IntC<ut>{}, IntC<slot_t>{}, IntC<H * half + decltype(ic)::value>{}); });
            };
            auto between = [&](auto gc) __attribute__((always_inline)) {
                constexpr int g = decltype(gc)::value;
                if constexpr (r == 3 && g >= 2) batch_pieces(IntC<5>{}, IntC<g - 2>{});
                else if constexpr (r == 0 && g < 2) batch_pieces(IntC<5>{}, IntC<g>{});
                else if constexpr (r == 0 && g >= 2) batch_pieces(IntC<6>{}, IntC<g - 2>{});
                else if constexpr (r == 1 && g < 2) batch_pieces(IntC<6>{}, IntC<g>{});
            };
            auto next = [&](auto jc) __attribute__((always_inline)) {
                constexpr int j = decltype(jc)::value;
                if constexpr (r == 3 && j == 5) landed();
                else if constexpr (r == 0 && j == 5) __builtin_amdgcn_s_barrier();
            };
            if constexpr (u < 8) {
                if constexpr (u == 0) {
#pragma unroll
                    for (int rt = 0; rt < RT; ++rt)
#pragma unroll
                        for (int j = 0; j < 8; ++j) hacc[rt][j] = f32x4{0.f, 0.f, 0.f, 0.f};
                }
                s16x8 bh[RT], bl[RT];
#pragma unroll
                for (int rt = 0; rt < RT; ++rt) { bh[rt] = xh[rt][u]; bl[rt] = xl[rt][u]; }
                stage_mma(IntC<slot>{}, hacc, IntC<0>{}, bh, bl, between, next);
            } else {
                constexpr int v = u - 8, c = v >> 1, nh = v & 1;
                if constexpr (nh == 0) {
                    const f32x4 ba = ld4(b1s + 128 * hs + 32 * c + 8 * fk), bb = ld4(b1s + 128 * hs + 32 * c + 8 * fk + 4);
#pragma unroll
                    for (int rt = 0; rt < RT; ++rt) {
                        f32x4 va, vb;
#pragma unroll
                        for (int e = 0; e < 4; ++e) {
                            if constexpr (DIAG == 4) { va[e] = hacc[rt][2 * c][e] + ba[e]; vb[e] = hacc[rt][2 * c + 1][e] + bb[e]; }
                            else { va[e] = gelu_erf(hacc[rt][2 * c][e] + ba[e]); vb[e] = gelu_erf(hacc[rt][2 * c + 1][e] + bb[e]); }
                        }
                        split8(va, vb, hh[rt][c], hl[rt][c]);
                    }
                }
                s16x8 bh[RT], bl[RT];
#pragma unroll
                for (int rt = 0; rt < RT; ++rt) { bh[rt] = hh[rt][c]; bl[rt] = hl[rt][c]; }
                stage_mma(IntC<slot>{}, oacc, IntC<8 * nh>{}, bh, bl, between, next);
            }
        });
    }
    wait_vm<0>();
    if constexpr (DIAG == 6) {
        wait_lgkm<0>(dummy[0][0], dummy[0][1], dummy[1][0], dummy[1][1]);
        wait_lgkm<0>(dummy[2][0], dummy[2][1], dummy[3][0], dummy[3][1]);
    } else if constexpr (DIAG != 3) {
        wait_lgkm<0>(wt[0][0], wt[0][1], wt[1][0], wt[1][1]);
        wait_lgkm<0>(wt[2][0], wt[2][1], wt[3][0], wt[3][1]);
    }

    if constexpr (DIAG == 5) {
        float s = 0.f;
#pragma unroll
        for (int rt = 0; rt < RT; ++rt)
#pragma unroll
            for (int jj = 0; jj < 16; ++jj) s += oacc[rt][jj][0] + oacc[rt][jj][1] + oacc[rt][jj][2] + oacc[rt][jj][3];
        if (live[0] && p.y != nullptr) p.y[(size_t)myrow[0] * D + fk] = s;
        return;
    }
    __syncthreads();
    char* const stg = lds + wave * 16384;
#pragma unroll
    for (int rt = 0; rt < RT; ++rt) {
        const size_t rbase = (size_t)myrow[rt] * D;
        f32x4 (&v)[16] = oacc[rt];
        float s = 0.f;
#pragma unroll
        for (int jj = 0; jj < 16; ++jj) {
            const int col = 32 * (jj >> 1) + 8 * fk + 4 * (jj & 1);
            const f32x4 bv = ld4(prm + col), rv = ld4(p.x + rbase + col);
#pragma unroll
            for (int e = 0; e < 4; ++e) { v[jj][e] = v[jj][e] + bv[e] + rv[e]; }
            s += (v[jj][0] + v[jj][1]) + (v[jj][2] + v[jj][3]);
        }
#pragma unroll
        for (int pass = 0; pass < 2; ++pass) {
            if (pass == 1 && p.g4 == nullptr) break;
            const float* gp = prm + (pass == 0 ? 1 : 3) * D;
            const float* bp = prm + (pass == 0 ? 2 : 4) * D;
            if (pass == 1) {
                s = 0.f;
#pragma unroll
                for (int jj = 0; jj < 16; ++jj) s += (v[jj][0] + v[jj][1]) + (v[jj][2] + v[jj][3]);
            }
            s += __shfl_xor(s, 16, 64); s += __shfl_xor(s, 32, 64);
            const float mean = s * (1.f / 256.f);
            float q = 0.f;
#pragma unroll
            for (int jj = 0; jj < 16; ++jj)
#pragma unroll
                for (int e = 0; e < 4; ++e) { const float d = v[jj][e] - mean; q = fmaf(d, d, q); }
            q += __shfl_xor(q, 16, 64); q += __shfl_xor(q, 32, 64);
            const float rstd = rsqrtf(q * (1.f / 256.f) + LN_EPS);
#pragma unroll
            for (int jj = 0; jj < 16; ++jj) {
                const int col = 32 * (jj >> 1) + 8 * fk + 4 * (jj & 1);
                const f32x4 ga = ld4(gp + col), be = ld4(bp + col);
#pragma unroll
                for (int e = 0; e < 4; ++e) v[jj][e] = (v[jj][e] - mean) * rstd * ga[e] + be[e];
            }
        }
#pragma unroll
        for (int jj = 0; jj < 16; ++jj) {
            const int ch = 8 * (jj >> 1) + 2 * fk + (jj & 1);
            *reinterpret_cast<f32x4*>(stg + frow * 1024 + ((ch ^ frow) << 4)) = v[jj];
        }
        const int row0 = blockIdx.x * BM + RW * wave + 16 * rt;
#pragma unroll
        for (int r = 0; r < 16; ++r) {
            const f32x4 o = *reinterpret_cast<const f32x4*>(stg + r * 1024 + ((lane ^ r) << 4));
            if (row0 + r < M) {
                if (p.y != nullptr) st4(p.y + (size_t)(row0 + r) * D + 4 * lane, o);
                if (p.ys != nullptr) store_split4(p.ys + (size_t)(row0 + r) * D, 4 * lane, o);
            }
        }
    }
}

std::atomic<int> g_mlp_variant{0};

int dec_mlp_prepare() {
    static std::mutex mu;
    static bool attr_set[64] = {};
    int dev = 0;
    LADIFF_HIP(hipGetDevice(&dev));
    if (dev < 0 || dev >= 64) return LADIFF_ERR_ARG;
    std::lock_guard<std::mutex> lock(mu);
    if (!attr_set[dev]) {
        const void* k[3] = {reinterpret_cast<const void*>(dec_mlp_kernel<4, 2>), reinterpret_cast<const void*>(dec_mlp_kernel<8, 1>),
                            reinterpret_cast<const void*>(dec_mlp_kernel<4, 1>)};
        for (int i = 0; i < 3; ++i) LADIFF_HIP(hipFuncSetAttribute(k[i], hipFuncAttributeMaxDynamicSharedMemorySize, MLP_LDS));
#ifdef LADIFF_STAMPS
        const void* d[7] = {reinterpret_cast<const void*>(dec_mlp_kernel<4, 2, 1>), reinterpret_cast<const void*>(dec_mlp_kernel<4, 2, 2>),
                            reinterpret_cast<const void*>(dec_mlp_kernel<4, 2, 3>), reinterpret_cast<const void*>(dec_mlp_kernel<4, 2, 4>),
                            reinterpret_cast<const void*>(dec_mlp_kernel<4, 2, 5>), reinterpret_cast<const void*>(dec_mlp_kernel<4, 2, 6>),
                            reinterpret_cast<const void*>(dec_mlp_kernel<4, 2, 7>)};
        for (int i = 0; i < 7; ++i) LADIFF_HIP(hipFuncSetAttribute(d[i], hipFuncAttributeMaxDynamicSharedMemorySize, MLP_LDS));
#endif
        attr_set[dev] = true;
    }
    return 0;
}
int dec_mlp_min_rows() { return 10000; }

int launch_dec_mlp(const float* xs, const float* x, const float* w1, const float* b1, const float* w2, const float* b2, const float* g3,
                   const float* be3, const float* g4, const float* be4, float* y, float* ys, int M, hipStream_t s) {
    if (M <= 0) return 0;
    LADIFF_TRY(dec_mlp_prepare());
    MlpArgs a{xs, x, w1, b1, w2, b2, g3, be3, g4, be4, y, ys, M};
    int form = g_mlp_variant;
    if (form >= 21) form = 0;
    if (form == 0) form = (M + 127) / 128 < 160 ? 2 : 1;
#ifdef LADIFF_STAMPS
    if (form >= 11 && form <= 17) {
        const void* k[7] = {reinterpret_cast<const void*>(dec_mlp_kernel<4, 2, 1>), reinterpret_cast<const void*>(dec_mlp_kernel<4, 2, 2>),
                            reinterpret_cast<const void*>(dec_mlp_kernel<4, 2, 3>), reinterpret_cast<const void*>(dec_mlp_kernel<4, 2, 4>),
                            reinterpret_cast<const void*>(dec_mlp_kernel<4, 2, 5>), reinterpret_cast<const void*>(dec_mlp_kernel<4, 2, 6>),
                            reinterpret_cast<const void*>(dec_mlp_kernel<4, 2, 7>)};
        void* args[] = {&a};
        LADIFF_HIP(hipLaunchKernel(k[form - 11], dim3((M + 127) / 128), dim3(256), args, MLP_LDS, s));
    } else
#endif
    if (form == 3) hipLaunchKernelGGL((dec_mlp_kernel<4, 2>), dim3((M + 127) / 128), dim3(256), MLP_LDS, s, a);
    else if (form == 1) hipLaunchKernelGGL((dec_mlp_kernel<8, 1>), dim3((M + 127) / 128), dim3(512), MLP_LDS, s, a);
    else hipLaunchKernelGGL((dec_mlp_kernel<4, 1>), dim3((M + 63) / 64), dim3(256), MLP_LDS, s, a);
    LADIFF_LAUNCH_CHECK();
    return 0;
}

}
```

ladiff_amd/csrc/decoder.hip:

```cpp
#include "model.h"
#ifdef LADIFF_STAMPS
#include <cstdlib>
#endif

namespace ladiff {

#ifdef LADIFF_STAMPS
#define DEC_CUT() do { if (dec_cut >= 0 && ++dec_launched >= dec_cut) return 0; } while (0)
#else
#define DEC_CUT() do { } while (0)
#endif

constexpr int DEC_SMALL_ROWS = 4096;
std::atomic<int> g_dec_out_cross{1};
std::atomic<int> g_dec_fused_attn{1};
std::atomic<int> g_dec_final_split{1};
std::atomic<int> g_dec_small_rows_path{1};
std::atomic<int> g_dec_fused_mlp{1};

static GemmArgs lin(const float* A, int lda, const float* W, const float* bias, float* Y, int ldy, int M, int N, int K,
                    int act = ACT_NONE) {
    GemmArgs g;
    g.A = A; g.lda = lda; g.W = W; g.ldw = K; g.bias = bias; g.Y = Y; g.ldy = ldy; g.M = M; g.N = N; g.K = K; g.act = act;
    return g;
}

int vae_decode(const DecoderW& w, const DecoderW* wsp, const float* z, const int32_t* lengths, const int32_t* counts,
               const int32_t* row_off, int R, int B, int F, int T, int C, float* feats, float* ws, size_t ws_floats, hipStream_t s) {
    if (F < 1 || F > LADIFF_MAX_FRAMES || T < 1 || T > LADIFF_MAX_LATENTS || C < 1) return LADIFF_ERR_SHAPE;
    const bool ragged = row_off != nullptr;
    if (ragged && (R < 0 || (size_t)R > (size_t)B * F)) return LADIFF_ERR_SHAPE;
    const int M = ragged ? R : B * F;
    DecWs a = dec_layout(ws, B, (size_t)M, T);
    if (ws_floats < a.total) return LADIFF_ERR_WORKSPACE;
    if (M == 0) return 0;
#ifdef LADIFF_STAMPS
    const char* dec_cut_env = getenv("LADIFF_DEC_CUT");
    const int dec_cut = dec_cut_env ? atoi(dec_cut_env) : -1;
    int dec_launched = 0;
    if (dec_cut == 0) return 0;
#endif
    const bool sp = wsp != nullptr;
    if (!sp) { for (float*& t : a.Ps) t = nullptr; for (float*& t : a.SKs) t = nullptr; }
    float *const *P = a.P, *const *SK = a.SK, *const *Ps = a.Ps, *const *SKs = a.SKs;
    float *qkv = a.qkv, *att = a.att, *hid = a.hid, *kv = a.kv, *guws = a.guws, *pex = a.pex, *pexs = a.pexs, *qkv0 = a.qkv0;
    int32_t* row_out = a.row_out;
    const size_t kv_l = a.kv_layer, gu_l = a.gu_layer;

    {
        GemmArgs g[NL];
        DecCrossPrepBatch pb;
        for (int l = 0; l < NL; ++l) {
            const DecLayerW& L = w.layer[l];
            g[l] = lin(z, D, L.cross_attn.in_w + (size_t)D * D, L.cross_attn.in_b + D, kv + l * kv_l, 2 * D, T * B, 2 * D, D);
            pb.kv[l] = kv + l * kv_l; pb.wq[l] = L.cross_attn.in_w; pb.bq[l] = L.cross_attn.in_b; pb.wo[l] = L.cross_attn.out_w;
            pb.gu[l] = guws + l * gu_l;
        }
        LADIFF_TRY(launch_gemm_batch(g, NL, s)); DEC_CUT();
        LADIFF_TRY(launch_decoder_cross_prep(pb, NL, B, T, s)); DEC_CUT();
    }

    const bool small = sp && M < DEC_SMALL_ROWS && g_dec_small_rows_path;
    const bool fused_attn = sp && g_dec_fused_attn && (M >= DEC_SMALL_ROWS || g_dec_fused_attn == 2);
    auto krs = [&](const float* A, int K, const float* W, const float* bias, float* Y, float* Ys, int ldy, int N, int act,
                   const float* res, int rows) -> int {
        KrArgs g;
        g.A = A; g.lda = K; g.W = W; g.ldw = K; g.bias = bias; g.Y = Y; g.Ys = Ys; g.ldy = ldy; g.M = rows; g.N = N; g.K = K; g.act = act;
        g.res = res; g.ldres = D; g.split = 1;
        return launch_gemm_kr(g, s);
    };

    auto gemm_ln = [&](const float* A, int K, const float* W, const float* Wsp, const float* bias, const float* res,
                       const NormW& n1, const NormW* n2, float* dst, float* dsts) -> int {
        GemmArgs g = lin(A, K, sp ? Wsp : W, bias, dst, D, M, D, K);
        g.res = res; g.ldres = D;
        if (!sp) {
            g.ln_g = n1.g; g.ln_b = n1.b;
            if (n2) { g.ln2_g = n2->g; g.ln2_b = n2->b; }
            return launch_gemm(g, s);
        }
        g.split = 1;
        LADIFF_TRY(launch_gemm(g, s));
        if (n2)
            return launch_reduce_rows(dst, 1, M, nullptr, nullptr, RED_LN, n1.g, n1.b, nullptr, 0, nullptr, nullptr, 1, 1, 0,
                                      0, dst, dsts, s, nullptr, n2->g, n2->b);
        return launch_reduce_rows(dst, 1, M, nullptr, nullptr, RED_LN, n1.g, n1.b, nullptr, 0, nullptr, nullptr, 1, 1, 0, 0,
                                  dst, dsts, s);
    };

    if (ragged) { LADIFF_TRY(launch_broadcast_pe_ragged(w.query_pe, row_off, B, F, F, P[0], Ps[0], row_out, s)); DEC_CUT(); }
    else { LADIFF_TRY(launch_broadcast_pe(w.query_pe, B, F, P[0], Ps[0], s)); DEC_CUT(); }
    const float* cur = P[0]; const float* curs = Ps[0];
    for (int l = 0; l < NL; ++l) {
        const DecLayerW& L = w.layer[l];
        const DecLayerW& Ls = sp ? wsp->layer[l] : w.layer[l];
        const bool is_in = l < NSKIP, is_out = l > NSKIP, last = l == NL - 1;
        if (is_out) {
            const LinearW& sk = w.skip[l - NSKIP - 1];
            if (small) {
                RowLnArgs g;
                g.A = curs; g.lda = D; g.A2 = SKs[NL - 1 - l]; g.lda2 = D; g.K1 = D; g.W = wsp->skip[l - NSKIP - 1].w; g.ldw = 2 * D; g.bias = sk.b;
                g.Y = P[3]; g.Ys = Ps[3]; g.ldy = D; g.M = M; g.K = 2 * D;
                LADIFF_TRY(launch_gemm_rowln(g, s)); DEC_CUT();
            } else {
            GemmArgs g = lin(sp ? curs : cur, D, sp ? wsp->skip[l - NSKIP - 1].w : sk.w, sk.b, P[3], D, M, D, 2 * D);
            g.A2 = sp ? SKs[NL - 1 - l] : SK[NL - 1 - l]; g.lda2 = D; g.K1 = D;
            g.split = sp ? 1 : 0; g.Ys = Ps[3];
            LADIFF_TRY(launch_gemm(g, s)); DEC_CUT();
            }
            cur = P[3]; curs = Ps[3];
        }
        const bool shared = l == 0;
        if (shared) {
            LADIFF_TRY(launch_broadcast_pe(w.query_pe, 1, F, pex, sp ? pexs : nullptr, s)); DEC_CUT();
            if (small) { LADIFF_TRY(krs(pexs, D, Ls.self_attn.in_w, L.self_attn.in_b, qkv0, nullptr, 3 * D, 3 * D, ACT_NONE, nullptr, F)); DEC_CUT(); }
            else {
            GemmArgs g = lin(sp ? pexs : pex, D, Ls.self_attn.in_w, L.self_attn.in_b, qkv0, 3 * D, F, 3 * D, D);
            g.split = sp ? 1 : 0;
            LADIFF_TRY(launch_gemm(g, s)); DEC_CUT();
            }
        } else if (fused_attn) {
        } else if (small) {
            LADIFF_TRY(krs(curs, D, Ls.self_attn.in_w, L.self_attn.in_b, qkv, nullptr, 3 * D, 3 * D, ACT_NONE, nullptr, M)); DEC_CUT();
        } else {
            GemmArgs g = lin(sp ? curs : cur, D, Ls.self_attn.in_w, L.self_attn.in_b, qkv, 3 * D, M, 3 * D, D);
            g.split = sp ? 1 : 0;
            LADIFF_TRY(launch_gemm(g, s)); DEC_CUT();
        }
        const float* qkv_l = shared ? qkv0 : qkv;
        if (fused_attn && !shared) { LADIFF_TRY(launch_dec_qkv_attn(curs, Ls.self_attn.in_w, L.self_attn.in_b, lengths, row_off, att, B, F, 1, s)); DEC_CUT(); }
        else if (sp) { LADIFF_TRY(launch_self_attention_split(qkv_l, lengths, nullptr, att, B, F, H, 0, 1, s, row_off, shared)); DEC_CUT(); }
        else { LADIFF_TRY(launch_decoder_self_attention(qkv_l, lengths, nullptr, att, B, F, 0, s, row_off, shared)); DEC_CUT(); }
        const NormW* n1_late = nullptr;
        if (sp && !small && g_dec_out_cross) {
            LADIFF_TRY(launch_decoder_out_cross(att, cur, Ls.self_attn.out_w, L.self_attn.out_b, L.norm1.g, L.norm1.b, L.cross_attn.out_b,
                                                L.norm2.g, L.norm2.b, counts, B, F, T, guws + l * gu_l, P[2], Ps[2], s, row_off)); DEC_CUT();
        } else {
        if (sp) {
            if (small) { LADIFF_TRY(krs(att, D, Ls.self_attn.out_w, L.self_attn.out_b, P[1], nullptr, D, D, ACT_NONE, cur, M)); DEC_CUT(); }
            else {
            GemmArgs g = lin(att, D, Ls.self_attn.out_w, L.self_attn.out_b, P[1], D, M, D, D);
            g.res = cur; g.ldres = D; g.split = 1;
            LADIFF_TRY(launch_gemm(g, s)); DEC_CUT();
            }
            n1_late = &L.norm1;
        } else {
            LADIFF_TRY(gemm_ln(att, D, L.self_attn.out_w, Ls.self_attn.out_w, L.self_attn.out_b, cur, L.norm1, nullptr, P[1], nullptr)); DEC_CUT();
        }
        LADIFF_TRY(launch_decoder_cross_apply(P[1], L.cross_attn.out_b, L.norm2.g, L.norm2.b, counts, B, F, T, guws + l * gu_l, P[2],
                                              Ps[2], s, row_off, n1_late ? n1_late->g : nullptr, n1_late ? n1_late->b : nullptr)); DEC_CUT();
        }
        float* dst = is_in ? SK[l] : P[0];
        float* dsts = is_in ? SKs[l] : Ps[0];
        if (sp && g_dec_fused_mlp && (M >= dec_mlp_min_rows() || g_dec_fused_mlp == 2)) {
            LADIFF_TRY(launch_dec_mlp(Ps[2], P[2], Ls.lin1.w, L.lin1.b, Ls.lin2.w, L.lin2.b, L.norm3.g, L.norm3.b,
                                      last ? w.norm.g : nullptr, last ? w.norm.b : nullptr, dst, dsts, M, s)); DEC_CUT();
        } else if (small) {
            LADIFF_TRY(krs(Ps[2], D, Ls.lin1.w, L.lin1.b, nullptr, hid, FF, FF, ACT_GELU, nullptr, M)); DEC_CUT();
            LADIFF_TRY(krs(hid, FF, Ls.lin2.w, nullptr, qkv, nullptr, D, D, ACT_NONE, nullptr, M)); DEC_CUT();
            LADIFF_TRY(launch_reduce_rows(qkv, 4, M, L.lin2.b, P[2], RED_LN, L.norm3.g, L.norm3.b, nullptr, 0, nullptr, nullptr, 1, 1, 0, 0,
                                          dst, dsts, s, nullptr, last ? w.norm.g : nullptr, last ? w.norm.b : nullptr));
        } else {
            GemmArgs g = lin(sp ? Ps[2] : P[2], D, Ls.lin1.w, L.lin1.b, sp ? nullptr : hid, FF, M, FF, D, ACT_GELU);
            g.split = sp ? 1 : 0; if (sp) g.Ys = hid;
            LADIFF_TRY(launch_gemm(g, s)); DEC_CUT();
            LADIFF_TRY(gemm_ln(hid, FF, L.lin2.w, Ls.lin2.w, L.lin2.b, P[2], L.norm3, last ? &w.norm : nullptr, dst, dsts)); DEC_CUT();
        }
        cur = dst; curs = dsts;
    }
    if (sp && M >= DEC_SMALL_ROWS && g_dec_final_split) {
        const int Np = (C + 127) / 128 * 128;
        if ((size_t)M * Np > a.hid_floats || (size_t)Np * (D + 1) > a.qkv_floats) return LADIFF_ERR_SHAPE;
        float* wpad = qkv; float* bpad = qkv + (size_t)Np * D;
        LADIFF_TRY(launch_pad_rows(wsp->final_layer.w, w.final_layer.b, wpad, bpad, C, Np, s)); DEC_CUT();
        GemmArgs g = lin(curs, D, wpad, bpad, hid, Np, M, Np, D);
        g.split = 1;
        LADIFF_TRY(launch_gemm(g, s)); DEC_CUT();
        return launch_scatter_feats(hid, Np, C, M, F, ragged ? nullptr : lengths, ragged ? row_out : nullptr, feats, s);
    }
    GemmArgs g = lin(cur, D, w.final_layer.w, w.final_layer.b, feats, C, M, C, D);
    if (ragged) g.row_map = row_out;
    else { g.row_len = lengths; g.rows_per_item = F; }
    return launch_gemm(g, s);
}

}
```

ladiff_amd/csrc/kernels.h:

```cpp
#pragma once
#include "common.h"
#include "noise_gen.h"

namespace ladiff {

enum RedMode : int { RED_PLAIN = 0, RED_LN = 1, RED_LN_ADD = 2, RED_LN_MOD = 3 };
int launch_reduce_rows(const float* P, int S, int M, const float* bias, const float* res, int mode, const float* g,
                       const float* b, const float* tab, int tab_step_stride, const int32_t* d_step,
                       const int32_t* counts, int Bs, int T, int pad_row, int b_off, float* out, float* outs, hipStream_t s,
                       const int32_t* d_base = nullptr, const float* g2 = nullptr, const float* b2 = nullptr);
int launch_split_rows(const float* x, float* y, int R, int K, hipStream_t s);
int launch_gather_rows(const float* src, const int32_t* index, int n_rows, int row_floats, float* dst, hipStream_t s);
int launch_split_range_stats(const float* const* xs, const int64_t* counts, int n, int64_t max_count, unsigned long long* stats,
                             hipStream_t s);
int launch_layernorm(const float* x, const float* g, const float* b, float* y, int M, hipStream_t s);
constexpr int DEC_PREP_MAX = 9;
struct DecCrossPrepBatch { const float* kv[DEC_PREP_MAX]; const float* wq[DEC_PREP_MAX]; const float* bq[DEC_PREP_MAX];
                           const float* wo[DEC_PREP_MAX]; float* gu[DEC_PREP_MAX]; };
constexpr int ROW_BATCH_MAX = 9;
struct RowBatch { const float* a[ROW_BATCH_MAX]; const float* g[ROW_BATCH_MAX]; const float* b[ROW_BATCH_MAX]; float* y[ROW_BATCH_MAX]; };
int launch_layernorm_batch(const RowBatch& rb, int n, int M, hipStream_t s);
int launch_ca_table_input_batch(const RowBatch& rb, int n_layers, int step_stride, int n, int B2, hipStream_t s, int split_out = 0);
int launch_ca_table_input(const float* nval, const float* beta, const float* mod, int step_stride, int n, int B2, float* u,
                          hipStream_t s);
int launch_add_pe(const float* sample, const float* pe, int Bs, int b_off, int b_n, int T, float* x, float* xs, hipStream_t s);
int launch_broadcast_pe(const float* pe, int B, int F, float* x, float* xs, hipStream_t s);
int launch_broadcast_pe_ragged(const float* pe, const int32_t* row_off, int B, int F, int F_out, float* x, float* xs, int32_t* row_out,
                               hipStream_t s);
int launch_relu(const float* x, float* y, size_t n, hipStream_t s);
int launch_pad_rows(const float* src, const float* srcb, float* dst, float* dstb, int C, int Np, hipStream_t s);
int launch_zero_fill(float* x, size_t n, hipStream_t s);
int launch_silu(const float* x, float* y, size_t n, hipStream_t s);
int launch_sinusoid(const int64_t* t, int n, float* out, hipStream_t s);
int launch_cfg_step(const float* eps, float* lat, const float* coef, const int32_t* d_step, const float* noise,
                    float g, int cfg, int B, int T, hipStream_t s);
int launch_advance(int32_t* d_step, hipStream_t s);
int launch_step_tail(float* x, float* xs, const float* ng, const float* nb, float* lat, const float* coef, int32_t* d_step,
                     const float* noise, const float* pe, float g, int cfg, int B, int T, hipStream_t s, const NoiseGen& gen = NoiseGen{0u, 0u, 0u, 0});
int launch_noise_fill(const NoiseGen& gen, int step0, int n, int B, int T, float* out, hipStream_t s);
int launch_init_latents(const float* noise, const int32_t* counts, float sigma, float* lat, int B, int T, hipStream_t s);
int launch_finalize_latents(const float* lat, const int32_t* counts, float* z, int B, int T, hipStream_t s, const unsigned* status = nullptr);

int launch_dec_qkv_attn(const float* xs, const float* w, const float* bias, const int32_t* lengths, const int32_t* row_off, float* out,
                        int B, int F, int split_out, hipStream_t s);
int launch_scatter_feats(const float* tmp, int ldt, int C, int M, int F, const int32_t* row_len, const int32_t* row_map, float* feats,
                         hipStream_t s);
int launch_pad_cols(const float* x, float* y, int R, int C, int Cp, hipStream_t s);
int launch_dvae_pad_cols(const float* x, const int32_t* slot, const float* values, int n, float* y, int B, int F, int C, int Cp,
                         hipStream_t s);
int launch_encoder_assemble(const float* token, const float* emb, const float* pe, const int32_t* lengths,
                            const int32_t* counts, int B, int F, int T, float* x, float* xs, uint32_t* keybits, hipStream_t s);
int launch_encoder_finalize(const float* out, const float* eps, const int32_t* counts, int B, int T, int S, float* mu, float* sd,
                            float* latent, hipStream_t s);

int launch_lca_kv(const float* key, const float* value, int B, int N, float* att, hipStream_t s);
int launch_lca_apply(const float* q, const float* att, const int32_t* counts, int Bs, int b_off, int b_n, int T, const float* mod,
                     int step_stride, int sample_stride, const int32_t* d_step, const float* g, const float* be, float* u,
                     hipStream_t s);
int launch_denoiser_self_attention_general(const float* qkv, const float* text_kv, int N, const float* tables, int kv_off,
                                           int step_stride, const int32_t* d_step, const int32_t* counts, int Bs, int b_off,
                                           int b_n, int T, float* out, hipStream_t s);

int launch_decoder_cross_prep(const DecCrossPrepBatch& pb, int n, int B, int T, hipStream_t s);
int launch_decoder_out_cross(const float* att_s, const float* x0, const float* wo_s, const float* bo, const float* g1, const float* b1,
                             const float* bo_c, const float* g2, const float* b2, const int32_t* counts, int B, int F, int T,
                             const float* gu_ws, float* y, float* ys, hipStream_t s, const int32_t* row_off);
int launch_decoder_cross_apply(const float* x, const float* bo, const float* g2, const float* b2, const int32_t* counts, int B, int F,
                               int T, const float* gu_ws, float* y, float* ys, hipStream_t s, const int32_t* row_off = nullptr,
                               const float* g1 = nullptr, const float* b1 = nullptr);

int launch_feats2joints(const float* feats, const float* mean, const float* stdv, int B, int F, int C, int J, float* joints,
                        hipStream_t s);

int launch_joint_ape_ave(const float* rst, const float* ref, const int32_t* lengths, int B, int F, int J, const int32_t* part_idx,
                         float factor, float* seq_rows, double* acc, hipStream_t s);
int launch_joint_mr(const float* rst, const float* ref, int B, int F, int J, float* seq_rows, double* acc, hipStream_t s);

int launch_vae_losses(const float* m_rst, const float* m_ref, size_t n_feat, const float* j_rst, const float* j_ref, size_t n_joint,
                      const float* mu, const float* sd, size_t n_lat, double l_rec, double l_joint, double l_kl, double* part, int blocks,
                      double* batch, double* acc, hipStream_t s);

int launch_denoiser_self_attention(const float* qkv, const float* text_kv, const float* tables, int kv_off,
                                   int step_stride, const int32_t* d_step, const int32_t* counts, int Bs, int b_off,
                                   int b_n, int T, float* out, int split_out, hipStream_t s);
int launch_decoder_self_attention(const float* qkv, const int32_t* lengths, const uint32_t* keybits, float* out, int B, int F,
                                  int split_out, hipStream_t s, const int32_t* row_off = nullptr, int shared_qkv = 0);
int launch_self_attention(const float* qkv, const int32_t* lengths, const uint32_t* keybits, float* out, int B, int F, int nheads,
                          int causal, int split_out, hipStream_t s, const int32_t* row_off = nullptr);
int launch_self_attention_split(const float* qkv, const int32_t* lengths, const uint32_t* keybits, float* out, int B, int F,
                                 int nheads, int causal, int split_out, hipStream_t s, const int32_t* row_off = nullptr, int shared_qkv = 0);
int launch_decoder_cross_attention(const float* q, const float* kv, const int32_t* counts, float* out, int B, int F,
                                   int T, int split_out, hipStream_t s);

}
```

ladiff_amd/csrc/model.h:

```cpp
#pragma once
#include <atomic>
#include "gemm.h"
#include "gemm_kr.h"
#include "graph_key.h"
#include "kernels.h"
#include "systolic_plan.h"
#include "weights.h"
#include "workspace.h"

namespace ladiff {

int denoiser_time_tables(const DenoiserW& w, const float* sinus, int n, float* tables, float* ws, size_t ws_floats, hipStream_t s);
int denoiser_text_cache(const DenoiserW& w, const float* text, int B2, const float* tables, int n_steps, float* cache,
                        float* ws, size_t ws_floats, hipStream_t s, int ntxt = 1);
int denoiser_forward(const DenoiserW& w, const DenoiserW* w_split, const float* tables, const int32_t* d_step,
                     const float* cache, int n_steps, const float* sample, int Bs, int dup, int T, const int32_t* counts, float* eps, float* ws,
                     size_t ws_floats, hipStream_t s, int b_lo = 0, int b_n = -1, int loop_mode = 0, int ntxt = 1,
                     const int32_t* d_base = nullptr);
int denoiser_text_static(const DenoiserW& w, const float* text, int B2, float* cache, float* ws, size_t ws_floats, hipStream_t s);
int denoiser_ctab(const DenoiserW& w, const float* tables_lo, int n, float* cache, int B2, float* u, size_t u_floats, hipStream_t s,
                  const DenoiserW* w_split = nullptr);
int linear_cross_attention(const DenoiserW& w, int layer, const float* x, const float* xf, const float* emb, const int32_t* counts,
                           int B, int T, int N, float* out, float* ws, size_t ws_floats, hipStream_t s);

int denoiser_forward_timesteps(const DenoiserW& w, const DenoiserW* w_split, const float* text, const int64_t* timesteps, const float* sample,
                               int B2, int T, const int32_t* counts, float* eps, float* ws, size_t ws_floats, hipStream_t s);
int launch_q_sample(const float* z, const int64_t* ts, const float* acp, int n_train, const int32_t* counts, const NoiseGen& gen, float* noise,
                    float* noisy, int B, int T, hipStream_t s);
int launch_diffusion_losses(const float* pred, const float* noise, size_t n, double lambda_inst, double* part, int blocks, double* batch,
                            double* acc, hipStream_t s);

struct Sampler;
int diffusion_reverse(Sampler* sp, const DenoiserW& w, const DenoiserW* w_split, const ReverseArgs& a);

extern std::atomic<int> g_dec_fused_mlp;
extern std::atomic<int> g_dec_small_rows_path;
extern std::atomic<int> g_dec_final_split;
extern std::atomic<int> g_dec_out_cross;
extern std::atomic<int> g_stage_plan;
extern std::atomic<int> g_poll_pause;
extern std::atomic<int> g_stage_delay;
extern std::atomic<int> g_pace;
extern std::atomic<int> g_look_ahead_from, g_small_upto;
extern std::atomic<int> g_dec_fused_attn;
extern std::atomic<int> g_mlp_variant;
int dec_mlp_prepare();
int dec_qkv_attn_prepare();
int dec_cross_prepare();
int dec_mlp_min_rows();
int vae_decode(const DecoderW& w, const DecoderW* w_split, const float* z, const int32_t* lengths, const int32_t* counts,
               const int32_t* row_off, int R, int B, int F, int T, int C, float* feats, float* ws, size_t ws_floats, hipStream_t s);

int launch_dec_mlp(const float* xs, const float* x, const float* w1, const float* b1, const float* w2, const float* b2, const float* g3,
                   const float* be3, const float* g4, const float* be4, float* y, float* ys, int M, hipStream_t s);

int vae_encode(const EncoderW& w, const EncoderW* w_split, const float* features, const int32_t* lengths,
               const int32_t* counts, const float* eps, int B, int F, int T, int C, float* mu, float* sd, float* latent, float* ws,
               size_t ws_floats, hipStream_t s, const int32_t* slot = nullptr, const float* values = nullptr, int n_values = 0);

#ifdef LADIFF_STAMPS
extern unsigned long long* g_sys_stamps;
extern int g_sys_probe;
#endif
bool sys_supported(int B, int T, int cfg, bool split);
extern std::atomic<int> g_waves16;
extern std::atomic<int> g_handoff;
int sys_reset_status(float* ws, hipStream_t s);
extern std::atomic<int> g_xcd_local;
int sys_build_stages(const DenoiserW& W, const DenoiserW& WS, float* ws, int MR, int NB, std::vector<unsigned char>& host);
int launch_systolic_loop(const DenoiserW& W, float* ws, const float* tables, const float* tkv, const float* ctab, int n_ctab,
                         const float* coef, const float* noise, float* lat, const int32_t* counts, float gscale, int B, int T,
                         int step_lo, int n, int fp32, int MR, int NB, hipStream_t s, int cfg = 1, int fault_wg = -1,
                         unsigned long long timeout_ticks = 0, const NoiseGen& gen = NoiseGen{0u, 0u, 0u, 0});

int launch_qkv_attention(const float* x, const float* w, const float* bias, const float* text_kv, const float* tables,
                         int kv_off, int step_stride, const int32_t* d_step, const int32_t* counts, int Bs, int b_off,
                         int b_n, int T, float* out, hipStream_t s);

int clip_text_encode(const ClipW& w, const ClipW* w_split, int n_layers, int vocab, const int64_t* ids, int B, int S, int L,
                     float* out, float* ws, size_t ws_floats, hipStream_t s, const int32_t* seq_len = nullptr,
                     const int32_t* row_off = nullptr, const int32_t* row_seq = nullptr, int total_rows = 0);

const std::vector<std::string>& t2m_move_param_names();
const std::vector<std::string>& t2m_motion_param_names();
const std::vector<std::string>& t2m_text_param_names();
int t2m_movement_encode(const float* const* w, const float* feats, int ld, int B, int F, int Cin, float* out, float* ws,
                        size_t ws_floats, hipStream_t s);
int t2m_motion_encode(const float* const* w, const float* mov, const int32_t* m_lens, int B, int T, float* out, float* ws,
                      size_t ws_floats, hipStream_t s);
int t2m_text_encode(const float* const* w, const float* word_embs, const float* pos_onehot, const int32_t* cap_lens, int B, int L,
                    float* out, float* ws, size_t ws_floats, hipStream_t s);

}
```

Baseline: 11190 motions/s.

## Add weight-streaming out-projection + cross-apply kernel for large decoder row counts

Moves the MLP kernel's LDS weight-streaming pipeline (global_load_lds DMA into an 8-slot ring, swizzled ds_read, split-bf16 MFMA) into a shared header. A new decoder out-projection/cross-attention-apply kernel uses it to stream the output weight through LDS, with each wave handling one 16-row tile. It is used when row_off is absent and B*F reaches the small-rows threshold. The existing out-cross kernel's chunk split also changes to spread 32-row passes evenly across the grid. The aim is to cut per-workgroup weight reload cost and raise MFMA throughput on large batches, at the price of a 512-thread kernel using much LDS and its own epilogue, which must match the old kernel's numerics.

```diff
diff --git a/ladiff_amd/build.py b/ladiff_amd/build.py
--- a/ladiff_amd/build.py
+++ b/ladiff_amd/build.py
@@ -7,7 +7,7 @@
 CSRC = os.path.join(HERE, "csrc")
 OBJ = os.path.join(HERE, "csrc", "build")
 LIB = os.path.join(HERE, "libladiff_hip.so")
-SOURCES = ["gemm.hip", "gemm_big.hip", "gemm_kr.hip", "gemm_rowln.hip", "rowops.hip", "attention.hip", "qkv_attn.hip", "systolic.hip", "systolic_plan.hip", "linear_ca.hip", "dec_cross.hip", "dec_mlp.hip", "dec_qkv_attn.hip", "feats2joints.hip", "joint_metrics.hip", "vae_losses.hip", "denoiser.hip", "diffusion_stage.hip", "decoder.hip", "encoder.hip", "clip.hip", "evaluator.hip", "reverse.hip", "api.hip"]
+SOURCES = ["gemm.hip", "gemm_big.hip", "gemm_kr.hip", "gemm_rowln.hip", "rowops.hip", "attention.hip", "qkv_attn.hip", "systolic.hip", "systolic_plan.hip", "linear_ca.hip", "dec_cross.hip", "dec_out_cross_stream.hip", "dec_mlp.hip", "dec_qkv_attn.hip", "feats2joints.hip", "joint_metrics.hip", "vae_losses.hip", "denoiser.hip", "diffusion_stage.hip", "decoder.hip", "encoder.hip", "clip.hip", "evaluator.hip", "reverse.hip", "api.hip"]
 FLAGS = ["--offload-arch=gfx950", "-O3", "-std=c++17", "-fPIC", "-fvisibility=hidden", "-Wall", "-Wno-unused-function"]
 
 
diff --git a/ladiff_amd/csrc/api.hip b/ladiff_amd/csrc/api.hip
--- a/ladiff_amd/csrc/api.hip
+++ b/ladiff_amd/csrc/api.hip
@@ -264,8 +264,9 @@
 }
 
 int ladiff_debug_set_decoder_fusion(int on) {
-    LADIFF_CHECK_ARG(on >= 0 && on <= 126 && (on & 3) != 3 && (on & 48) != 48);
+    LADIFF_CHECK_ARG(on >= 0 && on <= 254 && (on & 3) != 3 && (on & 48) != 48);
     g_dec_out_cross = (on & 64) ? 0 : 1;
+    g_dec_out_cross_stream = (on & 128) ? 0 : 1;
     g_dec_fused_mlp = on & 3;
     g_dec_small_rows_path = (on & 4) ? 0 : 1;
     g_dec_final_split = (on & 8) ? 0 : 1;
diff --git a/ladiff_amd/csrc/dec_cross.hip b/ladiff_amd/csrc/dec_cross.hip
--- a/ladiff_amd/csrc/dec_cross.hip
+++ b/ladiff_amd/csrc/dec_cross.hip
@@ -204,19 +204,6 @@
 constexpr int OC_SLD = 36;
 constexpr int OC_PS = 8 * OC_ROWS * OC_SLD * 4;
 constexpr int OC_PT = OC_ROWS * 256;
-
-struct OutCrossArgs {
-    const float* att;
-    const float* x0;
-    const float* wo;
-    const float* bo; const float* g1; const float* b1;
-    const float* gu; const float* cc;
-    const float* bo_c; const float* g2; const float* b2;
-    const int32_t* counts; const int32_t* row_off;
-    float* y; float* ys;
-    int F, rows_per_wg;
-    unsigned long long* stamps;
-};
 
 #ifdef LADIFF_STAMPS
 #define OC_STAMP(i) do { if (p.stamps != nullptr && blockIdx.x == 3 && blockIdx.y == 0 && threadIdx.x == 0 && npass < 6) p.stamps[npass * 16 + (i)] = __builtin_amdgcn_s_memrealtime(); } while (0)
@@ -305,8 +292,10 @@
     int F = p.F;
     size_t row0 = (size_t)b * F;
     if (p.row_off != nullptr) { row0 = p.row_off[b]; F = p.row_off[b + 1] - p.row_off[b]; }
-    const int f0 = blockIdx.y * p.rows_per_wg;
-    const int f1 = f0 + p.rows_per_wg < F ? f0 + p.rows_per_wg : F;
+    const int npasses = (F + OC_ROWS - 1) / OC_ROWS, nchunks = gridDim.y;
+    const int f0 = OC_ROWS * (npasses * (int)blockIdx.y / nchunks);
+    const int f1e = OC_ROWS * (npasses * ((int)blockIdx.y + 1) / nchunks);
+    const int f1 = f1e < F ? f1e : F;
     if (f0 >= f1) return;
     const int l16 = lane & 15, grp = lane >> 4, c0 = 4 * l16, lr = 4 * wave + grp;
     typedef unsigned u32x4_o __attribute__((ext_vector_type(4)));
@@ -510,7 +499,7 @@
             (void)oc[t - 1];
         attr_set[dev] = true;
     }
-    return 0;
+    return dec_out_cross_stream_prepare();
 }
 
 int launch_decoder_cross_prep(const DecCrossPrepBatch& pb, int n, int B, int T, hipStream_t s) {
@@ -555,16 +544,19 @@
 
 int launch_decoder_out_cross(const float* att_s, const float* x0, const float* wo_s, const float* bo, const float* g1, const float* b1,
                              const float* bo_c, const float* g2, const float* b2, const int32_t* counts, int B, int F, int T,
-                             const float* gu_ws, float* y, float* ys, hipStream_t s, const int32_t* row_off) {
+                             const float* gu_ws, float* y, float* ys, hipStream_t s, const int32_t* row_off, int stream_from_rows) {
     if (B == 0 || F == 0) return 0;
     if (T < 1 || T > TM) return LADIFF_ERR_SHAPE;
+    if (row_off == nullptr && stream_from_rows >= 0 && (long long)B * F >= stream_from_rows) {
+        LADIFF_TRY(dec_cross_prepare());
+        OutCrossArgs a{att_s, x0, wo_s, bo, g1, b1, gu_ws, gu_ws + (size_t)B * H * T * 2 * D, bo_c, g2, b2, counts, nullptr, y, ys, F, nullptr};
+        return launch_decoder_out_cross_stream(a, B, T, s);
+    }
     int chunks = (256 + B - 1) / B;
     if (chunks > (F + OC_ROWS - 1) / OC_ROWS) chunks = (F + OC_ROWS - 1) / OC_ROWS;
     if (chunks < 1) chunks = 1;
-    const int rows_per_wg = ((F + chunks - 1) / chunks + OC_ROWS - 1) / OC_ROWS * OC_ROWS;
-    chunks = (F + rows_per_wg - 1) / rows_per_wg;
     LADIFF_TRY(dec_cross_prepare());
-    OutCrossArgs a{att_s, x0, wo_s, bo, g1, b1, gu_ws, gu_ws + (size_t)B * H * T * 2 * D, bo_c, g2, b2, counts, row_off, y, ys, F, rows_per_wg, nullptr};
+    OutCrossArgs a{att_s, x0, wo_s, bo, g1, b1, gu_ws, gu_ws + (size_t)B * H * T * 2 * D, bo_c, g2, b2, counts, row_off, y, ys, F, nullptr};
 #ifdef LADIFF_STAMPS
     a.stamps = g_sys_stamps;
 #endif
diff --git a/ladiff_amd/csrc/dec_mlp.hip b/ladiff_amd/csrc/dec_mlp.hip
--- a/ladiff_amd/csrc/dec_mlp.hip
+++ b/ladiff_amd/csrc/dec_mlp.hip
@@ -1,17 +1,13 @@
 #include <mutex>
 #include "model.h"
-#include "tile_mma.h"
+#include "weight_stream.h"
 
 namespace ladiff {
 
 namespace {
 
-constexpr int MLP_NS = 8;
-constexpr int MLP_GRP = 4;
-constexpr int MLP_STAGE = 16384;
+constexpr int MLP_NS = WS_NS, MLP_GRP = WS_GRP, MLP_STAGE = WS_STAGE;
 constexpr int MLP_LDS = MLP_NS * MLP_STAGE + FF * 4 + 5 * D * 4;
-
-typedef unsigned u32x4_m __attribute__((ext_vector_type(4)));
 
 struct MlpArgs {
     const float* xs;
@@ -26,23 +22,6 @@
     int M;
 };
 
-__device__ __forceinline__ int pi_row(int p) { const int j = p >> 4, n = p & 15; return 32 * (j >> 1) + 8 * (n >> 2) + 4 * (j & 1) + (n & 3); }
-
-template <int N> __device__ __forceinline__ void wait_vm() { asm volatile("s_waitcnt vmcnt(%0)" ::"n"(N) : "memory"); }
-template <int OFF>
-__device__ __forceinline__ void fetch16(u32x4_m& v, unsigned addr) {
-    asm volatile("ds_read_b128 %0, %1 offset:%2" : "=v"(v) : "v"(addr), "n"(OFF) : "memory");
-}
-template <int OFF>
-__device__ __forceinline__ void fetch16_keep(u32x4_m& v, unsigned addr) {
-    asm volatile("ds_read_b128 %0, %1 offset:%2" : "+v"(v) : "v"(addr), "n"(OFF) : "memory");
-}
-template <int N>
-__device__ __forceinline__ void wait_lgkm(u32x4_m& a, u32x4_m& b, u32x4_m& c, u32x4_m& d) {
-    asm volatile("s_waitcnt lgkmcnt(%4)" : "+v"(a), "+v"(b), "+v"(c), "+v"(d) : "n"(N));
-}
-__device__ __forceinline__ s16x8 as_bf(const u32x4_m v) { return __builtin_bit_cast(s16x8, v); }
-
 }
 
 template <int NW, int RT, int DIAG = 0>
@@ -80,12 +59,11 @@
         if (src != nullptr) st4(prm + 4 * i, ld4(src + 4 * c4));
     }
 
-    const int cs = (lane & 7) ^ ((lane >> 4) & 3) ^ (4 * (wave & 1));
-    const int koff = (cs < 4 ? cs * 4 : 32 + (cs - 4) * 4);
+    WS_DMA_KOFF(koff, wave, lane);
     int src[PPW];
 #pragma unroll
-    for (int i = 0; i < PPW; ++i) src[i] = pi_row(8 * (wave + NW * i) + (lane >> 3));
-    char* const dma_dst = lds + (8 * wave) * 128;
+    for (int i = 0; i < PPW; ++i) src[i] = ws_dma_src<NW>(wave, lane, i);
+    char* const dma_dst = WS_DMA_DST(lds, wave);
     auto issue = [&](int hs, auto uc, auto slotc, auto ic) __attribute__((always_inline)) {
         constexpr int u = decltype(uc)::value, slot = decltype(slotc)::value, i = decltype(ic)::value;
         const float* base; int ldw, n0, kb, half;
@@ -94,13 +72,10 @@
         else { constexpr int v = u - 8, c = v >> 1; base = p.w2; ldw = FF; n0 = 128 * (v & 1); kb = 2 * hsv + (c >> 1); half = c & 1; }
         const float* s0 = base + (size_t)(n0 + src[i]) * ldw + kb * 64 + half * 16 + koff;
         if constexpr (DIAG == 1) { if (hs >= 0) return; }
-        __builtin_amdgcn_global_load_lds(s0, (__attribute__((address_space(3))) void*)(dma_dst + slot * MLP_STAGE + 8 * NW * i * 128), 16, 0, 0);
+        ws_dma_request<NW, slot, i>(s0, dma_dst);
     };
 
-    const int sw = (frow >> 1) & 7;
-    const unsigned rd_hi = lds_addr(lds) + frow * 128 + ((fk ^ sw) << 4);
-    const unsigned rd_lo = lds_addr(lds) + frow * 128 + (((4 + fk) ^ sw) << 4);
-    const unsigned rd_hi2 = rd_hi + 4 * MLP_STAGE, rd_lo2 = rd_lo + 4 * MLP_STAGE;
+    WS_READ_ADDR(rd, lds, frow, fk);
 
     f32x4 hacc[RT][8], oacc[RT][16];
     s16x8 hh[RT][4], hl[RT][4];
@@ -116,40 +91,10 @@
         for (int i = 0; i < 4; ++i) { asm volatile("" : "=v"(wt[i][0])); asm volatile("" : "=v"(wt[i][1])); asm volatile("" : "=v"(dummy[i][0])); asm volatile("" : "=v"(dummy[i][1])); }
     }
     auto fetch_tile = [&](auto slotc, auto jc) __attribute__((always_inline)) {
-        constexpr int slot = decltype(slotc)::value, j = decltype(jc)::value;
-        if constexpr (DIAG == 3) return;
-        const unsigned ah = slot < 4 ? rd_hi : rd_hi2, al = slot < 4 ? rd_lo : rd_lo2;
-        constexpr int so = (slot & 3) * MLP_STAGE;
-        if constexpr (DIAG == 6) { fetch16_keep<so + j * 2048>(dummy[j & 3][0], ah); fetch16_keep<so + j * 2048>(dummy[j & 3][1], al); return; }
-        fetch16<so + j * 2048>(wt[j & 3][0], ah); fetch16<so + j * 2048>(wt[j & 3][1], al);
+        ws_fetch_tile<DIAG, decltype(slotc)::value, decltype(jc)::value>(rd, wt, dummy);
     };
     auto stage_mma = [&](auto slotc, auto& acc, auto j0c, const s16x8 (&bh)[RT], const s16x8 (&bl)[RT], auto&& between, auto&& next) __attribute__((always_inline)) {
-        constexpr int slot = decltype(slotc)::value, J0 = decltype(j0c)::value;
-        static_for<8>([&](auto jc) {
-            constexpr int j = decltype(jc)::value, cur = j & 3;
-            next(jc);
-            if constexpr (DIAG != 3 && DIAG != 6) asm volatile("s_waitcnt lgkmcnt(4)" : "+v"(wt[cur][0]), "+v"(wt[cur][1]));
-            __builtin_amdgcn_sched_barrier(0);
-            static_for<3 * RT>([&](auto mc) {
-                constexpr int m = decltype(mc)::value, prod = m / RT, rt = m % RT;
-                if constexpr (DIAG == 7) {
-                    acc[rt][J0 + j] = MFMA16_S16(as_bf(dummy[cur][prod == 1]), prod == 0 ? bl[rt] : bh[rt], acc[rt][J0 + j], 0, 0, 0);
-                } else if constexpr (DIAG != 2) {
-                    if constexpr (prod == 0) acc[rt][J0 + j] = MFMA16_S16(as_bf(wt[cur][0]), bl[rt], acc[rt][J0 + j], 0, 0, 0);
-                    else if constexpr (prod == 1) acc[rt][J0 + j] = MFMA16_S16(as_bf(wt[cur][1]), bh[rt], acc[rt][J0 + j], 0, 0, 0);
-                    else acc[rt][J0 + j] = MFMA16_S16(as_bf(wt[cur][0]), bh[rt], acc[rt][J0 + j], 0, 0, 0);
-                }
-                if constexpr (m == 0) {
-                    __builtin_amdgcn_sched_barrier(0);
-                    if constexpr (j + 3 < 8) fetch_tile(slotc, IntC<j + 3>{});
-                    else fetch_tile(IntC<(slot + 1) % MLP_NS>{}, IntC<j + 3 - 8>{});
-                    __builtin_amdgcn_sched_barrier(0);
-                }
-            });
-            if constexpr (DIAG == 2) acc[0][J0 + j][0] += __builtin_bit_cast(float, wt[cur][0][0]) + __builtin_bit_cast(float, wt[cur][1][1]);
-            __builtin_amdgcn_sched_barrier(0);
-            if constexpr (j & 1) between(IntC<j / 2>{});
-        });
+        ws_stage_mma<DIAG, RT, decltype(slotc)::value, decltype(j0c)::value>(rd, wt, dummy, acc, bh, bl, between, next);
     };
 
     static_for<MLP_GRP>([&](auto uc) {
@@ -157,11 +102,7 @@
         static_for<PPW>([&](auto ic) { issue(DIAG == 1 ? -1 : 0, IntC<u>{}, IntC<u>{}, ic); });
     });
     __syncthreads();
-    auto landed = [&]() __attribute__((always_inline)) {
-        wait_vm<0>();
-        __builtin_amdgcn_s_barrier();
-    };
-    landed();
+    ws_landed();
     static_for<PPW>([&](auto ic) { issue(DIAG == 1 ? -1 : 0, IntC<MLP_GRP>{}, IntC<MLP_GRP>{}, ic); });
     static_for<3>([&](auto jc) { fetch_tile(IntC<0>{}, jc); });
     constexpr int H = PPW / 2;
@@ -177,15 +118,10 @@
             };
             auto between = [&](auto gc) __attribute__((always_inline)) {
                 constexpr int g = decltype(gc)::value;
-                if constexpr (r == 3 && g >= 2) batch_pieces(IntC<5>{}, IntC<g - 2>{});
-                else if constexpr (r == 0 && g < 2) batch_pieces(IntC<5>{}, IntC<g>{});
-                else if constexpr (r == 0 && g >= 2) batch_pieces(IntC<6>{}, IntC<g - 2>{});
-                else if constexpr (r == 1 && g < 2) batch_pieces(IntC<6>{}, IntC<g>{});
+                if constexpr (ws_batch_ahead<r, g>() != 0) batch_pieces(IntC<ws_batch_ahead<r, g>()>{}, IntC<ws_batch_half<r, g>()>{});
             };
             auto next = [&](auto jc) __attribute__((always_inline)) {
-                constexpr int j = decltype(jc)::value;
-                if constexpr (r == 3 && j == 5) landed();
-                else if constexpr (r == 0 && j == 5) __builtin_amdgcn_s_barrier();
+                ws_next<r, decltype(jc)::value>();
             };
             if constexpr (u < 8) {
                 if constexpr (u == 0) {
diff --git a/ladiff_amd/csrc/dec_out_cross_stream.hip b/ladiff_amd/csrc/dec_out_cross_stream.hip
--- /dev/null
+++ b/ladiff_amd/csrc/dec_out_cross_stream.hip
@@ -0,0 +1,257 @@
+#include <mutex>
+#include "kernels.h"
+#include "weight_stream.h"
+
+namespace ladiff {
+
+namespace {
+constexpr int OCS_NW = 8, OCS_PPW = 16 / OCS_NW;
+constexpr int OCS_LDS = WS_NS * WS_STAGE + 6 * D * 4;
+}
+
+template <int TT>
+__global__ __launch_bounds__(64 * OCS_NW, 2) void dec_out_cross_stream_kernel(const OutCrossArgs p, int ntiles, int tps) {
+    constexpr int NW = OCS_NW, PPW = OCS_PPW, NT = 64 * NW, HT = H * TT, NJT = TT > 4 ? 2 : 1;
+    static_assert(TT >= 1 && TT <= 8, "a head's tokens fit the eight k values of a lane group");
+    extern __shared__ __attribute__((aligned(1024))) char lds[];
+    float* const vec = reinterpret_cast<float*>(lds + WS_NS * WS_STAGE);
+    const int tid = threadIdx.x, lane = tid & 63;
+    const int wave = __builtin_amdgcn_readfirstlane(tid >> 6);
+    const int frow = lane & 15, fk = lane >> 4;
+    const int tile_id = blockIdx.x * NW + wave;
+    const bool active = tile_id < ntiles;
+    const int tile = active ? tile_id : ntiles - 1;
+    const int b = tile / tps, r0 = (tile - b * tps) * 16;
+    const int F = p.F;
+    const bool live = r0 + frow < F;
+    const size_t row = (size_t)b * F + (live ? r0 + frow : F - 1);
+
+    s16x8 xh[8], xl[8];
+    {
+        const char* xr = reinterpret_cast<const char*>(p.att) + row * 1024 + fk * 16;
+#pragma unroll
+        for (int s = 0; s < 8; ++s) {
+            xh[s] = *reinterpret_cast<const s16x8*>(xr + (s >> 1) * 256 + (s & 1) * 64);
+            xl[s] = *reinterpret_cast<const s16x8*>(xr + (s >> 1) * 256 + (s & 1) * 64 + 128);
+        }
+    }
+    for (int i = tid; i < 6 * D / 4; i += NT) {
+        const int which = i / (D / 4), c4 = i % (D / 4);
+        const float* src = which == 0 ? p.bo : which == 1 ? p.g1 : which == 2 ? p.b1 : which == 3 ? p.bo_c : which == 4 ? p.g2 : p.b2;
+        st4(vec + 4 * i, ld4(src + 4 * c4));
+    }
+
+    WS_DMA_KOFF(koff, wave, lane);
+    int src[PPW];
+#pragma unroll
+    for (int i = 0; i < PPW; ++i) src[i] = ws_dma_src<NW>(wave, lane, i);
+    char* const dma_dst = WS_DMA_DST(lds, wave);
+    auto issue = [&](auto uc, auto ic) __attribute__((always_inline)) {
+        constexpr int u = decltype(uc)::value, i = decltype(ic)::value, n0 = 128 * (u >> 3), s = u & 7;
+        const float* s0 = p.wo + (size_t)(n0 + src[i]) * D + (s >> 1) * 64 + (s & 1) * 16 + koff;
+        ws_dma_request<NW, u % WS_NS, i>(s0, dma_dst);
+    };
+    WS_READ_ADDR(rd, lds, frow, fk);
+
+    f32x4 acc[1][16];
+#pragma unroll
+    for (int j = 0; j < 16; ++j) acc[0][j] = f32x4{0.f, 0.f, 0.f, 0.f};
+    u32x4_m wt[4][2];
+
+    static_for<WS_GRP>([&](auto uc) { static_for<PPW>([&](auto ic) { issue(uc, ic); }); });
+    __syncthreads();
+    ws_landed();
+    static_for<PPW>([&](auto ic) { issue(IntC<WS_GRP>{}, ic); });
+    static_for<3>([&](auto jc) { ws_fetch_tile<0, 0, decltype(jc)::value>(rd, wt, wt); });
+    static_for<16>([&](auto uc) {
+        constexpr int u = decltype(uc)::value, slot = u % WS_NS, r = u % WS_GRP;
+        auto between = [&](auto gc) __attribute__((always_inline)) {
+            constexpr int g = decltype(gc)::value, ahead = ws_batch_ahead<r, g>();
+            if constexpr (ahead != 0 && u + ahead < 16) issue(IntC<u + ahead>{}, IntC<ws_batch_half<r, g>()>{});
+        };
+        auto next = [&](auto jc) __attribute__((always_inline)) { ws_next<r, decltype(jc)::value>(); };
+        const s16x8 bh[1] = {xh[u & 7]}, bl[1] = {xl[u & 7]};
+        ws_stage_mma<0, 1, slot, 8 * (u >> 3)>(rd, wt, wt, acc, bh, bl, between, next);
+    });
+    wait_vm<0>();
+    wait_lgkm<0>(wt[0][0], wt[0][1], wt[1][0], wt[1][1]);
+    wait_lgkm<0>(wt[2][0], wt[2][1], wt[3][0], wt[3][1]);
+    __syncthreads();
+    if (!active) return;
+
+    f32x4 (&v)[16] = acc[0];
+    const float* const vb = vec + 8 * fk;
+    auto ccol = [](int jj) { return 32 * (jj >> 1) + 4 * (jj & 1); };
+    auto layer_norm = [&](auto gwc) __attribute__((always_inline)) {
+        constexpr int gw = decltype(gwc)::value;
+        float s = 0.f;
+#pragma unroll
+        for (int jj = 0; jj < 16; ++jj) s += (v[jj][0] + v[jj][1]) + (v[jj][2] + v[jj][3]);
+        s += __shfl_xor(s, 16, 64); s += __shfl_xor(s, 32, 64);
+        const float mean = s * (1.f / 256.f);
+        float q = 0.f;
+#pragma unroll
+        for (int jj = 0; jj < 16; ++jj)
+#pragma unroll
+            for (int e = 0; e < 4; ++e) { const float d = v[jj][e] - mean; q = fmaf(d, d, q); }
+        q += __shfl_xor(q, 16, 64); q += __shfl_xor(q, 32, 64);
+        const float rstd = rsqrtf(q * (1.f / 256.f) + LN_EPS);
+#pragma unroll
+        for (int jj = 0; jj < 16; ++jj) {
+            const f32x4 ga = ld4(vb + D * gw + ccol(jj)), be = ld4(vb + D * (gw + 1) + ccol(jj));
+#pragma unroll
+            for (int e = 0; e < 4; ++e) v[jj][e] = (v[jj][e] - mean) * rstd * ga[e] + be[e];
+        }
+    };
+    const float* gub = p.gu + (size_t)b * HT * 2 * D;
+    const float* grow[NJT];
+#pragma unroll
+    for (int jt = 0; jt < NJT; ++jt) {
+        const int t = 4 * jt + (frow & 3);
+        grow[jt] = gub + (size_t)((frow >> 2) * TT + (t < TT ? t : TT - 1)) * 2 * D + 8 * fk;
+    }
+    f32x4 graw[8][NJT][2];
+    auto g_request = [&](int c0) __attribute__((always_inline)) {
+#pragma unroll
+        for (int c = c0; c < c0 + 4; ++c)
+#pragma unroll
+            for (int jt = 0; jt < NJT; ++jt) { graw[c][jt][0] = ld4(grow[jt] + 32 * c); graw[c][jt][1] = ld4(grow[jt] + 32 * c + 4); }
+    };
+    {
+        const float* xres = p.x0 + row * D;
+#pragma unroll
+        for (int jj = 0; jj < 16; ++jj) {
+            const f32x4 bv = ld4(vb + ccol(jj)), rv = ld4(xres + 8 * fk + ccol(jj));
+#pragma unroll
+            for (int e = 0; e < 4; ++e) v[jj][e] = (v[jj][e] + bv[e]) + rv[e];
+        }
+        layer_norm(IntC<1>{});
+    }
+
+    const float* ub = gub + ((size_t)fk * TT * 2 + 1) * D + 8 * (frow >> 2) + (frow & 3);
+    float uraw[16][TT];
+    auto u_request = [&](int j0) __attribute__((always_inline)) {
+#pragma unroll
+        for (int jj = j0; jj < j0 + 4; ++jj)
+#pragma unroll
+            for (int t = 0; t < TT; ++t) uraw[jj][t] = ub[(size_t)t * 2 * D + 32 * (jj >> 1) + 4 * (jj & 1)];
+    };
+
+    int nv = p.counts != nullptr ? p.counts[b] : TT;
+    nv = nv > TT ? TT : nv;
+    f32x4 sacc[NJT];
+#pragma unroll
+    for (int jt = 0; jt < NJT; ++jt) sacc[jt] = f32x4{0.f, 0.f, 0.f, 0.f};
+    g_request(0); g_request(4); u_request(0);
+    __builtin_amdgcn_sched_barrier(0);
+#pragma unroll
+    for (int c = 0; c < 8; ++c) {
+        s16x8 bh, bl;
+        split8(v[2 * c], v[2 * c + 1], bh, bl);
+#pragma unroll
+        for (int jt = 0; jt < NJT; ++jt) {
+            s16x8 gh, gl;
+            split8(graw[c][jt][0], graw[c][jt][1], gh, gl);
+            sacc[jt] = MFMA16_S16(gh, bl, sacc[jt], 0, 0, 0);
+            sacc[jt] = MFMA16_S16(gl, bh, sacc[jt], 0, 0, 0);
+            sacc[jt] = MFMA16_S16(gh, bh, sacc[jt], 0, 0, 0);
+        }
+    }
+    u_request(4);
+    __builtin_amdgcn_sched_barrier(0);
+    float pr[8];
+    {
+        const float* cb = p.cc + (size_t)b * HT + fk * TT;
+        float sc[4 * NJT];
+#pragma unroll
+        for (int t = 0; t < 4 * NJT; ++t) sc[t] = sacc[t >> 2][t & 3] + cb[t < TT ? t : TT - 1];
+        float m = -INFINITY, l = 0.f;
+#pragma unroll
+        for (int t = 0; t < 4 * NJT; ++t) if (t < TT) m = t < nv ? fmaxf(m, sc[t]) : m;
+#pragma unroll
+        for (int t = 0; t < 4 * NJT; ++t) {
+            const float e = t < TT ? __builtin_amdgcn_exp2f((sc[t] - m) * 1.4426950408889634f) : 0.f;
+            sc[t] = t < nv ? e : 0.f;
+            l += sc[t];
+        }
+#pragma unroll
+        for (int t = 0; t < 8; ++t) pr[t] = (t < TT && t < 4 * NJT) ? (t < nv ? sc[t < 4 * NJT ? t : 0] / l : 0.f) : 0.f;
+    }
+    {
+        s16x8 ph, pl;
+        split8(f32x4{pr[0], pr[1], pr[2], pr[3]}, f32x4{pr[4], pr[5], pr[6], pr[7]}, ph, pl);
+#pragma unroll
+        for (int jj = 0; jj < 16; ++jj) {
+            if (jj == 4 || jj == 8) { u_request(jj + 4); __builtin_amdgcn_sched_barrier(0); }
+            const f32x4 bc = ld4(vb + 3 * D + ccol(jj));
+            float uv[8];
+#pragma unroll
+            for (int t = 0; t < 8; ++t) uv[t] = 0.f;
+#pragma unroll
+            for (int t = 0; t < TT; ++t) uv[t] = uraw[jj][t];
+            s16x8 uh, ul;
+            split8(f32x4{uv[0], uv[1], uv[2], uv[3]}, f32x4{uv[4], uv[5], uv[6], uv[7]}, uh, ul);
+#pragma unroll
+            for (int e = 0; e < 4; ++e) v[jj][e] = bc[e] + v[jj][e];
+            v[jj] = MFMA16_S16(uh, pl, v[jj], 0, 0, 0);
+            v[jj] = MFMA16_S16(ul, ph, v[jj], 0, 0, 0);
+            v[jj] = MFMA16_S16(uh, ph, v[jj], 0, 0, 0);
+        }
+    }
+    layer_norm(IntC<4>{});
+
+    char* const stg = lds + wave * WS_STAGE;
+#pragma unroll
+    for (int jj = 0; jj < 16; ++jj) {
+        const int ch = 8 * (jj >> 1) + 2 * fk + (jj & 1);
+        *reinterpret_cast<f32x4*>(stg + frow * 1024 + ((ch ^ frow) << 4)) = v[jj];
+    }
+    const size_t orow0 = (size_t)b * F + r0;
+#pragma unroll
+    for (int r = 0; r < 16; ++r) {
+        const f32x4 o = *reinterpret_cast<const f32x4*>(stg + r * 1024 + ((lane ^ r) << 4));
+        if (r0 + r < F) {
+            if (p.y != nullptr) st4(p.y + (orow0 + r) * D + 4 * lane, o);
+            if (p.ys != nullptr) store_split4(p.ys + (orow0 + r) * D, 4 * lane, o);
+        }
+    }
+}
+
+int dec_out_cross_stream_prepare() {
+    static std::mutex mu;
+    static bool attr_set[64] = {};
+    int dev = 0;
+    LADIFF_HIP(hipGetDevice(&dev));
+    if (dev < 0 || dev >= 64) return LADIFF_ERR_ARG;
+    std::lock_guard<std::mutex> lock(mu);
+    if (!attr_set[dev]) {
+        const void* k[8] = {reinterpret_cast<const void*>(dec_out_cross_stream_kernel<1>), reinterpret_cast<const void*>(dec_out_cross_stream_kernel<2>),
+                            reinterpret_cast<const void*>(dec_out_cross_stream_kernel<3>), reinterpret_cast<const void*>(dec_out_cross_stream_kernel<4>),
+                            reinterpret_cast<const void*>(dec_out_cross_stream_kernel<5>), reinterpret_cast<const void*>(dec_out_cross_stream_kernel<6>),
+                            reinterpret_cast<const void*>(dec_out_cross_stream_kernel<7>), reinterpret_cast<const void*>(dec_out_cross_stream_kernel<8>)};
+        for (int i = 0; i < 8; ++i) LADIFF_HIP(hipFuncSetAttribute(k[i], hipFuncAttributeMaxDynamicSharedMemorySize, OCS_LDS));
+        attr_set[dev] = true;
+    }
+    return 0;
+}
+
+int launch_decoder_out_cross_stream(const OutCrossArgs& a, int B, int T, hipStream_t s) {
+    if (a.row_off != nullptr || T < 1 || T > LADIFF_MAX_LATENTS) return LADIFF_ERR_SHAPE;
+    const int tps = oc_stream_tiles_per_sample(a.F);
+    const long long nt = (long long)B * tps;
+    if (nt <= 0 || nt > 0x7fffffff - OCS_NW) return LADIFF_ERR_SHAPE;
+    const int ntiles = (int)nt;
+    LADIFF_TRY(dec_out_cross_stream_prepare());
+#define LADIFF_OCS_CASE(TT) \
+    case TT: hipLaunchKernelGGL(dec_out_cross_stream_kernel<TT>, dim3((ntiles + OCS_NW - 1) / OCS_NW), dim3(64 * OCS_NW), OCS_LDS, s, a, ntiles, tps); break;
+    switch (T) {
+        LADIFF_OCS_CASE(1) LADIFF_OCS_CASE(2) LADIFF_OCS_CASE(3) LADIFF_OCS_CASE(4)
+        LADIFF_OCS_CASE(5) LADIFF_OCS_CASE(6) LADIFF_OCS_CASE(7) LADIFF_OCS_CASE(8)
+        default: return LADIFF_ERR_SHAPE;
+    }
+#undef LADIFF_OCS_CASE
+    LADIFF_LAUNCH_CHECK();
+    return 0;
+}
+
+}
diff --git a/ladiff_amd/csrc/decoder.hip b/ladiff_amd/csrc/decoder.hip
--- a/ladiff_amd/csrc/decoder.hip
+++ b/ladiff_amd/csrc/decoder.hip
@@ -13,6 +13,7 @@
 
 constexpr int DEC_SMALL_ROWS = 4096;
 std::atomic<int> g_dec_out_cross{1};
+std::atomic<int> g_dec_out_cross_stream{1};
 std::atomic<int> g_dec_fused_attn{1};
 std::atomic<int> g_dec_final_split{1};
 std::atomic<int> g_dec_small_rows_path{1};
@@ -134,7 +135,8 @@
         const NormW* n1_late = nullptr;
         if (sp && !small && g_dec_out_cross) {
             LADIFF_TRY(launch_decoder_out_cross(att, cur, Ls.self_attn.out_w, L.self_attn.out_b, L.norm1.g, L.norm1.b, L.cross_attn.out_b,
-                                                L.norm2.g, L.norm2.b, counts, B, F, T, guws + l * gu_l, P[2], Ps[2], s, row_off)); DEC_CUT();
+                                                L.norm2.g, L.norm2.b, counts, B, F, T, guws + l * gu_l, P[2], Ps[2], s, row_off,
+                                                g_dec_out_cross_stream ? DEC_SMALL_ROWS : -1)); DEC_CUT();
         } else {
         if (sp) {
             if (small) { LADIFF_TRY(krs(att, D, Ls.self_attn.out_w, L.self_attn.out_b, P[1], nullptr, D, D, ACT_NONE, cur, M)); DEC_CUT(); }
diff --git a/ladiff_amd/csrc/kernels.h b/ladiff_amd/csrc/kernels.h
--- a/ladiff_amd/csrc/kernels.h
+++ b/ladiff_amd/csrc/kernels.h
@@ -62,9 +62,24 @@
                                            int b_n, int T, float* out, hipStream_t s);
 
 int launch_decoder_cross_prep(const DecCrossPrepBatch& pb, int n, int B, int T, hipStream_t s);
+struct OutCrossArgs {
+    const float* att;
+    const float* x0;
+    const float* wo;
+    const float* bo; const float* g1; const float* b1;
+    const float* gu; const float* cc;
+    const float* bo_c; const float* g2; const float* b2;
+    const int32_t* counts; const int32_t* row_off;
+    float* y; float* ys;
+    int F;
+    unsigned long long* stamps;
+};
 int launch_decoder_out_cross(const float* att_s, const float* x0, const float* wo_s, const float* bo, const float* g1, const float* b1,
                              const float* bo_c, const float* g2, const float* b2, const int32_t* counts, int B, int F, int T,
-                             const float* gu_ws, float* y, float* ys, hipStream_t s, const int32_t* row_off);
+                             const float* gu_ws, float* y, float* ys, hipStream_t s, const int32_t* row_off, int stream_from_rows);
+inline int oc_stream_tiles_per_sample(int F) { return (F + 15) / 16; }
+int launch_decoder_out_cross_stream(const OutCrossArgs& a, int B, int T, hipStream_t s);
+int dec_out_cross_stream_prepare();
 int launch_decoder_cross_apply(const float* x, const float* bo, const float* g2, const float* b2, const int32_t* counts, int B, int F,
                                int T, const float* gu_ws, float* y, float* ys, hipStream_t s, const int32_t* row_off = nullptr,
                                const float* g1 = nullptr, const float* b1 = nullptr);
diff --git a/ladiff_amd/csrc/model.h b/ladiff_amd/csrc/model.h
--- a/ladiff_amd/csrc/model.h
+++ b/ladiff_amd/csrc/model.h
@@ -37,6 +37,7 @@
 extern std::atomic<int> g_dec_small_rows_path;
 extern std::atomic<int> g_dec_final_split;
 extern std::atomic<int> g_dec_out_cross;
+extern std::atomic<int> g_dec_out_cross_stream;
 extern std::atomic<int> g_stage_plan;
 extern std::atomic<int> g_poll_pause;
 extern std::atomic<int> g_stage_delay;
diff --git a/ladiff_amd/csrc/weight_stream.h b/ladiff_amd/csrc/weight_stream.h
--- /dev/null
+++ b/ladiff_amd/csrc/weight_stream.h
@@ -0,0 +1,100 @@
+#pragma once
+#include "tile_mma.h"
+
+namespace ladiff {
+namespace {
+
+constexpr int WS_NS = 8;
+constexpr int WS_GRP = 4;
+constexpr int WS_STAGE = 16384;
+
+typedef unsigned u32x4_m __attribute__((ext_vector_type(4)));
+
+__device__ __forceinline__ int pi_row(int p) { const int j = p >> 4, n = p & 15; return 32 * (j >> 1) + 8 * (n >> 2) + 4 * (j & 1) + (n & 3); }
+
+template <int N> __device__ __forceinline__ void wait_vm() { asm volatile("s_waitcnt vmcnt(%0)" ::"n"(N) : "memory"); }
+template <int OFF>
+__device__ __forceinline__ void fetch16(u32x4_m& v, unsigned addr) {
+    asm volatile("ds_read_b128 %0, %1 offset:%2" : "=v"(v) : "v"(addr), "n"(OFF) : "memory");
+}
+template <int OFF>
+__device__ __forceinline__ void fetch16_keep(u32x4_m& v, unsigned addr) {
+    asm volatile("ds_read_b128 %0, %1 offset:%2" : "+v"(v) : "v"(addr), "n"(OFF) : "memory");
+}
+template <int N>
+__device__ __forceinline__ void wait_lgkm(u32x4_m& a, u32x4_m& b, u32x4_m& c, u32x4_m& d) {
+    asm volatile("s_waitcnt lgkmcnt(%4)" : "+v"(a), "+v"(b), "+v"(c), "+v"(d) : "n"(N));
+}
+__device__ __forceinline__ s16x8 as_bf(const u32x4_m v) { return __builtin_bit_cast(s16x8, v); }
+
+#define WS_DMA_KOFF(koff, wave, lane)                                                    \
+    const int koff##_cs = ((lane) & 7) ^ (((lane) >> 4) & 3) ^ (4 * ((wave) & 1));       \
+    const int koff = (koff##_cs < 4 ? koff##_cs * 4 : 32 + (koff##_cs - 4) * 4)
+template <int NW> __device__ __forceinline__ int ws_dma_src(int wave, int lane, int i) { return pi_row(8 * (wave + NW * i) + (lane >> 3)); }
+#define WS_DMA_DST(lds, wave) ((lds) + (8 * (wave)) * 128)
+template <int NW, int slot, int i>
+__device__ __forceinline__ void ws_dma_request(const float* s0, char* dma_dst) {
+    __builtin_amdgcn_global_load_lds(s0, (__attribute__((address_space(3))) void*)(dma_dst + slot * WS_STAGE + 8 * NW * i * 128), 16, 0, 0);
+}
+
+__device__ __forceinline__ void ws_landed() {
+    wait_vm<0>();
+    __builtin_amdgcn_s_barrier();
+}
+
+template <int r, int g> constexpr int ws_batch_ahead() {
+    return (r == 3 && g >= 2) ? 5 : (r == 0 && g < 2) ? 5 : (r == 0 && g >= 2) ? 6 : (r == 1 && g < 2) ? 6 : 0;
+}
+template <int r, int g> constexpr int ws_batch_half() { return ((r == 3 || r == 0) && g >= 2) ? g - 2 : g; }
+template <int r, int j> __device__ __forceinline__ void ws_next() {
+    if constexpr (r == 3 && j == 5) ws_landed();
+    else if constexpr (r == 0 && j == 5) __builtin_amdgcn_s_barrier();
+}
+
+struct WsRead { unsigned hi, lo, hi2, lo2; };
+#define WS_READ_ADDR(rd, lds, frow, fk)                                                              \
+    const int rd##_sw = ((frow) >> 1) & 7;                                                           \
+    const unsigned rd##_hi = lds_addr(lds) + (frow) * 128 + (((fk) ^ rd##_sw) << 4);                 \
+    const unsigned rd##_lo = lds_addr(lds) + (frow) * 128 + (((4 + (fk)) ^ rd##_sw) << 4);           \
+    const WsRead rd{rd##_hi, rd##_lo, rd##_hi + 4 * WS_STAGE, rd##_lo + 4 * WS_STAGE}
+template <int DIAG, int slot, int j>
+__device__ __forceinline__ void ws_fetch_tile(const WsRead& rd, u32x4_m (&wt)[4][2], u32x4_m (&dummy)[4][2]) {
+    if constexpr (DIAG == 3) return;
+    const unsigned ah = slot < 4 ? rd.hi : rd.hi2, al = slot < 4 ? rd.lo : rd.lo2;
+    constexpr int so = (slot & 3) * WS_STAGE;
+    if constexpr (DIAG == 6) { fetch16_keep<so + j * 2048>(dummy[j & 3][0], ah); fetch16_keep<so + j * 2048>(dummy[j & 3][1], al); return; }
+    fetch16<so + j * 2048>(wt[j & 3][0], ah); fetch16<so + j * 2048>(wt[j & 3][1], al);
+}
+
+template <int DIAG, int RT, int slot, int J0, class Acc, class Between, class Next>
+__device__ __forceinline__ void ws_stage_mma(const WsRead& rd, u32x4_m (&wt)[4][2], u32x4_m (&dummy)[4][2], Acc& acc, const s16x8 (&bh)[RT],
+                                             const s16x8 (&bl)[RT], Between&& between, Next&& next) {
+    static_for<8>([&](auto jc) {
+        constexpr int j = decltype(jc)::value, cur = j & 3;
+        next(jc);
+        if constexpr (DIAG != 3 && DIAG != 6) asm volatile("s_waitcnt lgkmcnt(4)" : "+v"(wt[cur][0]), "+v"(wt[cur][1]));
+        __builtin_amdgcn_sched_barrier(0);
+        static_for<3 * RT>([&](auto mc) {
+            constexpr int m = decltype(mc)::value, prod = m / RT, rt = m % RT;
+            if constexpr (DIAG == 7) {
+                acc[rt][J0 + j] = MFMA16_S16(as_bf(dummy[cur][prod == 1]), prod == 0 ? bl[rt] : bh[rt], acc[rt][J0 + j], 0, 0, 0);
+            } else if constexpr (DIAG != 2) {
+                if constexpr (prod == 0) acc[rt][J0 + j] = MFMA16_S16(as_bf(wt[cur][0]), bl[rt], acc[rt][J0 + j], 0, 0, 0);
+                else if constexpr (prod == 1) acc[rt][J0 + j] = MFMA16_S16(as_bf(wt[cur][1]), bh[rt], acc[rt][J0 + j], 0, 0, 0);
+                else acc[rt][J0 + j] = MFMA16_S16(as_bf(wt[cur][0]), bh[rt], acc[rt][J0 + j], 0, 0, 0);
+            }
+            if constexpr (m == 0) {
+                __builtin_amdgcn_sched_barrier(0);
+                if constexpr (j + 3 < 8) ws_fetch_tile<DIAG, slot, j + 3>(rd, wt, dummy);
+                else ws_fetch_tile<DIAG, (slot + 1) % WS_NS, j + 3 - 8>(rd, wt, dummy);
+                __builtin_amdgcn_sched_barrier(0);
+            }
+        });
+        if constexpr (DIAG == 2) acc[0][J0 + j][0] += __builtin_bit_cast(float, wt[cur][0][0]) + __builtin_bit_cast(float, wt[cur][1][1]);
+        __builtin_amdgcn_sched_barrier(0);
+        if constexpr (j & 1) between(IntC<j / 2>{});
+    });
+}
+
+}
+}
```

Result: no change. 11230 motions/s, median of 6 (+0.3%).
